# viridityzhu/HiFiHR

Measured on AMD Instinct MI355X. Metric: train images/sec, FreiHAND 224x224 (ResNet-18 + MANO LBS + render + losses + Adam), higher is better.
Workload: dtype f32; 1 GPU; BASELINE configs[1]: FreiHAND batch=32/GPU, ResNet-18 encoder + MANO LBS + silhouette/texture render losses, 224x224, aa=3 (672^2 samples); per_gpu_batch=32, global_batch=32, parallelism=dp1

## Files before the change

hifihr_amd/_lib.py:

```python
from __future__ import annotations

import ctypes
import os
from ctypes import POINTER, c_char_p, c_float, c_int, c_int32, c_long, c_size_t, c_void_p

import torch

_HERE = os.path.dirname(os.path.abspath(__file__))
LIB_PATH = os.path.join(_HERE, "libhifihr.so")

_c_float_p = POINTER(c_float)


class _LinearDesc(ctypes.Structure):
    _fields_ = [("x", c_void_p), ("w", c_void_p), ("b", c_void_p), ("y", c_void_p), ("B", c_int), ("I", c_int), ("O", c_int), ("act", c_int),
                ("dy", c_void_p), ("dz_scratch", c_void_p), ("dW_acc", c_void_p), ("db_acc", c_void_p), ("dx", c_void_p)]

_c_int_p = POINTER(c_int32)


class HifihrError(RuntimeError):
    pass


# ... 104 lines not shown
        c.hifihr_image_scale_to_nhwc4.argtypes = [_c_float_p, _c_float_p, c_int, c_int, c_int, _c_float_p, _c_float_p, c_void_p]
        c.hifihr_maxpool2d_fwd_notap.argtypes = [_c_float_p] + [c_int] * 7 + [_c_float_p, c_void_p]
        c.hifihr_lpips_tap_max_channels.argtypes = []
        c.hifihr_lpips_tap_max_channels.restype = c_int
        c.hifihr_lpips_tap_partial_floats.argtypes = [c_int]
        c.hifihr_lpips_tap_partial_floats.restype = c_size_t
        c.hifihr_lpips_tap.argtypes = [_c_float_p] * 3 + [c_int] * 4 + [_c_float_p, _c_float_p, c_void_p]
        c.hifihr_lpips_tap_bwd.argtypes = [_c_float_p] * 4 + [c_int] * 4 + [_c_float_p, c_void_p]
        c.hifihr_lpips_tap_bwd_relu.argtypes = [_c_float_p] * 4 + [c_int] * 4 + [_c_float_p, c_void_p]
        c.hifihr_lpips_maxpool_fwd.argtypes = [_c_float_p] + [c_int] * 4 + [_c_float_p, c_void_p]
        c.hifihr_lpips_maxpool_bwd.argtypes = [_c_float_p, _c_float_p] + [c_int] * 4 + [_c_float_p, c_void_p]
        c.hifihr_image_scale_to_nhwc4_bwd.argtypes = [_c_float_p, _c_float_p, c_int, c_int, c_int, _c_float_p, c_void_p]
        c.hifihr_geom_loss_fwd.argtypes = [_c_float_p] * 6 + [_c_int_p] + [c_int] * 7 + [_c_float_p] * 3 + [c_void_p]
        c.hifihr_geom_loss_bwd.argtypes = [_c_float_p] * 6 + [_c_int_p] * 3 + [c_int] * 7 + [_c_float_p] * 6 + [c_void_p]
        c.hifihr_photo_loss_partial_floats.argtypes = []
        c.hifihr_photo_loss_partial_floats.restype = c_int
        c.hifihr_photo_loss_fwd.argtypes = [_c_float_p, _c_float_p, c_void_p, c_int, c_int, c_int, c_float, c_float, c_float] + \
            [_c_float_p] * 4 + [c_void_p]
        c.hifihr_photo_loss_bwd.argtypes = [_c_float_p] * 6 + [c_int, c_int, c_int, c_float, c_float, _c_float_p, c_void_p]
        c.hifihr_sil_post.argtypes = [_c_float_p, _c_float_p, c_int, c_int, c_int, _c_float_p, _c_float_p, c_void_p]
        c.hifihr_linear_fwd.argtypes = [_c_float_p] * 3 + [c_int] * 4 + [_c_float_p] * 2 + [c_float, c_float] + [_c_float_p] * 6 + [c_void_p]
        c.hifihr_linear_bwd.argtypes = [_c_float_p] * 4 + [c_int] * 4 + [_c_float_p] * 10 + [c_void_p]
        c.hifihr_linear_fwd_group.argtypes = [POINTER(_LinearDesc), c_int, c_void_p]
        c.hifihr_linear_bwd_group.argtypes = [POINTER(_LinearDesc), c_int, c_void_p]
        c.hifihr_conv2d_bwd_data_pre.argtypes = [_c_float_p] * 3 + [c_int] * 9 + [c_void_p, c_size_t, c_void_p]
        c.hifihr_conv2d_bwd_data_pre_res.argtypes = [_c_float_p] * 4 + [c_int] * 9 + [c_void_p, c_size_t, c_void_p]
        c.hifihr_conv2d_bwd_data_pre_plus1x1.argtypes = [_c_float_p] * 5 + [c_int] * 9 + [c_void_p]
        c.hifihr_conv2d_bwd_data_pre_plus1x1_supported.argtypes = [c_int] * 9
        c.hifihr_conv2d_bwd_weight_plus1x1.argtypes = [_c_float_p] * 5 + [c_int] * 9 + [c_void_p]
        c.hifihr_conv2d_bwd_weight_plus1x1_supported.argtypes = [c_int] * 9
        c.hifihr_weight_prep.argtypes = [c_void_p, c_int, c_int, c_void_p]
        c.hifihr_freihand_augment.argtypes = [c_void_p, c_void_p, _c_int_p, _c_int_p, c_int, c_int, c_int, _c_float_p, _c_float_p, c_void_p]
        c.hifihr_ho3d_workspace_bytes.argtypes = [c_int, c_int]
        c.hifihr_ho3d_workspace_bytes.restype = c_size_t
        c.hifihr_ho3d_batch.argtypes = ([c_void_p, c_void_p] + [_c_float_p] * 3 + [c_int, c_int, _c_int_p, c_int, c_int, c_void_p, c_size_t] +
                                        [_c_float_p] * 5 + [c_void_p])
        c.hifihr_freihand_batch.argtypes = ([c_void_p, c_void_p] + [_c_float_p] * 4 + [c_int, c_int, _c_int_p, c_int, c_int, c_int, _c_float_p,
                                            _c_float_p, c_void_p] + [_c_float_p] * 6 + [c_void_p, c_void_p])
        c.hifihr_freihand_batch_step.argtypes = ([c_void_p, c_void_p] + [_c_float_p] * 4 + [c_int, c_int, _c_int_p, c_int, c_int, c_int, _c_float_p,
                                                 _c_float_p, c_void_p] + [_c_float_p] * 6 + [c_void_p, c_int, c_float] + [_c_float_p] * 4 + [c_void_p])
        c.hifihr_light_split_fwd.argtypes = [_c_float_p, c_int, _c_float_p, _c_float_p, c_void_p]
        c.hifihr_light_split_bwd.argtypes = [_c_float_p, _c_float_p, _c_float_p, c_int, _c_float_p, c_void_p]
        c.hifihr_wino4_bwd_gemm_pair_supported.argtypes = [c_int] * 5
        c.hifihr_wino4_bwd_gemm_pair.argtypes = [_c_float_p] * 6 + [c_int] * 6 + [c_void_p]
        c.hifihr_loss_total_fwd.argtypes = [POINTER(_c_float_p), POINTER(c_int), c_int, _c_float_p, c_void_p]
        c.hifihr_loss_total_bwd.argtypes = [_c_float_p, POINTER(_c_float_p), POINTER(c_int), POINTER(c_int), c_int, c_void_p]
        c.hifihr_procrustes_error.argtypes = [_c_float_p, _c_float_p, c_int, c_int, _c_float_p, _c_float_p, c_void_p]
        c.hifihr_point_error_hist.argtypes = [_c_float_p, _c_float_p, c_void_p, c_int, c_int, POINTER(ctypes.c_double), c_int, _c_int_p, c_void_p,
                                              c_void_p]
        c.hifihr_fscore_counts.argtypes = [_c_float_p, _c_float_p, c_int, c_int, c_int, POINTER(ctypes.c_double), c_int, _c_int_p, c_void_p]
        c.hifihr_wino_wgrad_gemm.argtypes = [_c_float_p] * 3 + [c_int] * 5 + [c_void_p]
        c.hifihr_wino_dw_transform.argtypes = [_c_float_p, _c_float_p, c_int, c_int, c_int, c_void_p]
        c.hifihr_weight_transpose.argtypes = [_c_float_p, _c_float_p, c_int, c_int, c_int, c_void_p]
        c.hifihr_bgemm_nt.argtypes = [_c_float_p] * 3 + [c_int] * 4 + [c_void_p, c_size_t, c_void_p]
        c.hifihr_bgemm_nt_workspace_bytes.argtypes = [c_int] * 4
        c.hifihr_bgemm_nt_workspace_bytes.restype = c_size_t
        c.hifihr_renderer_set_light_mode.argtypes = [c_void_p, c_int]
        c.hifihr_texture_pca_fwd.argtypes = [_c_float_p] * 3 + [c_int, c_int, c_long, _c_float_p, c_void_p]
        c.hifihr_texture_pca_bwd.argtypes = [_c_float_p] * 2 + [c_int, c_int, c_long, _c_float_p, c_void_p]
        c.hifihr_comm_last_error.restype = c_char_p
        c.hifihr_comm_get_unique_id.argtypes = [c_void_p]
        c.hifihr_comm_init.argtypes = [POINTER(c_void_p), c_int, c_int, c_void_p]
        c.hifihr_comm_allreduce_f32.argtypes = [c_void_p, _c_float_p, c_size_t, c_void_p]
        c.hifihr_comm_broadcast_f32.argtypes = [c_void_p, _c_float_p, c_size_t, c_int, c_void_p]
        c.hifihr_comm_destroy.argtypes = [c_void_p]
        c.hifihr_wino_tile.argtypes = [c_int] * 5
        c.hifihr_wino_gemm_workspace_bytes.argtypes = [c_int] * 6
        c.hifihr_wino_gemm_workspace_bytes.restype = c_size_t
        c.hifihr_wino_weight_transform.argtypes = [_c_float_p, _c_float_p, c_int, c_int, c_int, c_int, c_void_p]
        c.hifihr_wino_input_transform.argtypes = [_c_float_p, _c_float_p] + [c_int] * 5 + [c_void_p]
        c.hifihr_wino_gemm.argtypes = [_c_float_p] * 3 + [c_int] * 6 + [c_void_p, c_size_t, c_void_p]
        c.hifihr_wino_output_transform.argtypes = [_c_float_p] * 3 + [c_int] * 5 + [c_void_p]
        c.hifihr_wino_output_transform_act.argtypes = [_c_float_p] * 3 + [c_int] * 6 + [c_void_p]
        c.hifihr_conv3x3_c64_wino_supported.argtypes = [c_int] * 5
        c.hifihr_conv3x3_c64_wino.argtypes = [c_void_p, c_void_p, c_void_p, c_int, c_void_p, c_void_p, c_int, c_int, c_int, c_void_p]
        c.hifihr_conv3x3_c64_wino_res.argtypes = [c_void_p, c_void_p, c_void_p, c_void_p, c_int, c_int, c_int, c_void_p]
        c.hifihr_conv3x3_c64_bwd_pair_supported.argtypes = [c_int] * 3
        c.hifihr_conv3x3_c64_bwd_pair.argtypes = [c_void_p] * 7 + [c_size_t] + [c_int] * 3 + [c_void_p]
        c.hifihr_conv3x3_c64_bwd_pair_slabs.argtypes = [c_void_p] * 6 + [c_size_t] + [c_int] * 3 + [c_void_p, c_void_p]
        c.hifihr_conv_halo_wgrad_reduce_multi.argtypes = [c_void_p, c_int, c_void_p]
        c.hifihr_wino_bn_input_supported.argtypes = [c_int, c_int]
        c.hifihr_wino_bn_input_transform.argtypes = [_c_float_p] * 7 + [c_int] * 5 + [c_float, c_float] + [_c_float_p] * 4 + [c_void_p]
        c.hifihr_wino_output_transform_bnred.argtypes = [_c_float_p] * 10 + [c_int] * 5 + [c_void_p]
        c.hifihr_wino_bn_bwd_dual_transform.argtypes = [_c_float_p] * 8 + [c_int] * 5 + [_c_float_p] * 2 + [c_void_p]
        c.hifihr_bn_bwd_apply.argtypes = [_c_float_p] * 5 + [c_long, c_int] + [_c_float_p] * 4 + [c_void_p]
        c.hifihr_joint_terms_fwd.argtypes = [_c_float_p] * 4 + [c_int] * 3 + [POINTER(c_float), _c_float_p, c_void_p]
        c.hifihr_joint_terms_bwd.argtypes = [_c_float_p] * 4 + [c_int] * 3 + [POINTER(c_float)] + [_c_float_p] * 3 + [c_void_p]
        c.hifihr_wino_dy_transform.argtypes = [_c_float_p] * 2 + [c_int] * 5 + [c_void_p]
        c.hifihr_wino_input_dy_transform.argtypes = [_c_float_p] * 3 + [c_int] * 5 + [c_void_p]
        c.hifihr_wino_wgrad_parts.argtypes = [c_int] * 6
        c.hifihr_wino_wgrad_gemm_parts.argtypes = [_c_float_p] * 3 + [c_int] * 7 + [c_void_p]
        c.hifihr_wino_dw_transform_parts.argtypes = [_c_float_p, c_int, _c_float_p, c_int, c_int, c_int, c_void_p]
        c.hifihr_bgemm_describe.argtypes = [c_int] * 5 + [ctypes.c_char_p, c_int]
        c.hifihr_conv2d_describe.argtypes = [c_int] * 10 + [ctypes.c_char_p, c_int]
        c.hifihr_bgemm_tn_parts.argtypes = [c_int] * 4
        c.hifihr_bgemm_tn.argtypes = [_c_float_p] * 3 + [c_int] * 5 + [c_void_p]
        c.hifihr_wino4_dw_transform_multi.argtypes = [c_void_p, c_int, c_void_p]
        c.hifihr_se_pool.argtypes = [_c_float_p, c_int, c_int, c_int, _c_float_p, c_void_p]
        c.hifihr_se_scale.argtypes = [_c_float_p, _c_float_p, _c_float_p, c_float, c_int, c_int, c_int, _c_float_p, c_void_p]
        c.hifihr_se_bwd_gate.argtypes = [_c_float_p, _c_float_p, c_int, c_int, c_int, _c_float_p, c_void_p]
        c.hifihr_se_mlp_supported.argtypes = [c_int, c_int]
        c.hifihr_wino_tiles.argtypes = [c_int] * 4
        c.hifihr_wino_tiles.restype = c_long
        c.hifihr_wino_tiles_computed.argtypes = [c_int] * 4
        c.hifihr_wino_tiles_computed.restype = c_long
        c.hifihr_zero_page_ready.argtypes = [c_void_p]
        c.hifihr_drop_connect_add.argtypes = [_c_float_p, _c_float_p, _c_float_p, c_float, c_int, c_size_t, _c_float_p, c_void_p]
        c.hifihr_se_mlp_fwd.argtypes = [_c_float_p] * 5 + [c_int] * 3 + [_c_float_p] * 4 + [c_void_p]
        c.hifihr_se_mlp_bwd.argtypes = [_c_float_p] * 7 + [c_int] * 3 + [_c_float_p] * 7 + [c_void_p]
        c.hifihr_mmpool_fwd.argtypes = [_c_float_p, _c_float_p, c_int, c_int, c_int, _c_float_p, _c_int_p, _c_float_p, _c_float_p, c_void_p]
        c.hifihr_mmpool_bwd.argtypes = [_c_float_p, _c_float_p, _c_int_p, _c_float_p, _c_float_p, c_int, c_int, c_int, _c_float_p,
                                        _c_float_p, c_void_p]
        c.hifihr_maxpool2d_fwd.argtypes = [_c_float_p] + [c_int] * 7 + [_c_float_p, c_void_p, c_void_p]
        c.hifihr_maxpool2d_bwd.argtypes = [_c_float_p, c_void_p] + [c_int] * 7 + [_c_float_p, c_void_p]
        c.hifihr_maxpool2d_fwd_flat.argtypes = [_c_float_p] + [c_int] * 7 + [_c_float_p, c_void_p, c_void_p]
        c.hifihr_maxpool2d_bwd_flat.argtypes = [_c_float_p, c_void_p] + [c_int] * 7 + [_c_float_p, c_void_p]
        c.hifihr_maxpool2d_bwd_relu.argtypes = [_c_float_p, c_void_p, _c_float_p] + [c_int] * 7 + [_c_float_p, c_void_p]
        c.hifihr_wino_output_transform_mask.argtypes = [_c_float_p] * 3 + [c_int] * 5 + [c_void_p]
        c.hifihr_adam_step.argtypes = [_c_float_p, _c_float_p, _c_float_p, _c_float_p, c_size_t, c_float, c_float, c_float,
                                       c_float, c_float, c_float, c_int, c_void_p]
        c.hifihr_adam_state_bytes.restype = c_size_t
        c.hifihr_adam_state_bytes.argtypes = []
        c.hifihr_adam_step_counted.argtypes = [_c_float_p, _c_float_p, _c_float_p, _c_float_p, c_size_t, c_float, c_float, c_float, c_void_p, c_void_p]
        c.hifihr_grad_guard_bytes.restype = c_size_t
        c.hifihr_grad_guard_bytes.argtypes = []
        c.hifihr_grad_norm_workspace_bytes.restype = c_size_t
        c.hifihr_grad_norm_workspace_bytes.argtypes = [c_size_t]
        c.hifihr_grad_norm.argtypes = [_c_float_p, c_size_t, c_float, c_float, c_void_p, c_void_p, c_void_p]
        c.hifihr_adam_step_guarded.argtypes = [_c_float_p, _c_float_p, _c_float_p, _c_float_p, c_size_t, c_float, c_float, c_float, c_float,
                                               c_float, c_float, c_int, c_void_p, c_void_p, c_void_p]
        c.hifihr_adam_step_dyn.argtypes = [_c_float_p, _c_float_p, _c_float_p, _c_float_p, c_size_t, c_float, c_float, c_float,
                                           c_float, c_float, _c_float_p, c_void_p]
        c.hifihr_renderer_destroy.argtypes = [c_void_p]
        c.hifihr_render_workspace_bytes.argtypes = [c_void_p, c_int]
        c.hifihr_render_workspace_bytes.restype = c_size_t
        c.hifihr_render_fwd.argtypes = [c_void_p, _c_float_p, _c_float_p, c_int, _c_float_p, _c_float_p, _c_float_p, c_int,
                                        _c_float_p, _c_int_p, c_void_p, c_void_p]
        c.hifihr_render_bwd.argtypes = [c_void_p, _c_float_p, _c_float_p, _c_float_p, _c_float_p, _c_int_p, _c_float_p, c_int,
                                        _c_float_p, _c_float_p, _c_float_p, _c_float_p, c_void_p, c_void_p]
        c.hifihr_soft_sil_workspace_bytes.argtypes = [c_void_p, c_int]
        c.hifihr_soft_sil_workspace_bytes.restype = c_size_t
        c.hifihr_soft_sil_fwd.argtypes = [c_void_p, _c_float_p, _c_float_p, c_int, c_float, c_float, _c_float_p, _c_float_p, c_void_p, c_void_p]
        c.hifihr_soft_sil_bwd.argtypes = [c_void_p, _c_float_p, _c_float_p, _c_float_p, _c_float_p, c_int, c_float, c_float, _c_float_p, c_void_p,
                                          c_void_p]
        c.hifihr_soft_sil_loss_fwd.argtypes = [_c_float_p, c_void_p, c_int, c_int, c_int, c_float, c_float, c_void_p, _c_float_p, c_void_p]
        c.hifihr_soft_sil_loss_bwd.argtypes = [_c_float_p, c_void_p, c_int, c_void_p, _c_float_p, c_int, c_int, c_float, c_float, _c_float_p,
                                               c_void_p]
        c.hifihr_mesh_topology_create.argtypes = [_c_int_p, c_int, c_int]
        c.hifihr_mesh_topology_create.restype = c_void_p
        c.hifihr_mesh_topology_destroy.argtypes = [c_void_p]
        c.hifihr_mesh_topology_counts.argtypes = [c_void_p, _c_int_p, _c_int_p, _c_int_p]
        c.hifihr_mesh_reg_partial_floats.argtypes = [c_void_p, c_int]
        c.hifihr_mesh_reg_partial_floats.restype = c_size_t
        c.hifihr_mesh_reg_fwd.argtypes = [c_void_p, _c_float_p, c_int, c_float, c_float, _c_float_p, _c_float_p, _c_float_p, c_void_p]
        c.hifihr_mesh_reg_bwd.argtypes = [c_void_p, _c_float_p, _c_float_p, _c_float_p, c_int, c_float, c_float, _c_float_p, c_void_p]
        c.hifihr_chamfer_geometry.argtypes = [_c_int_p, _c_int_p]
        c.hifihr_chamfer_geometry.restype = None
        c.hifihr_chamfer_workspace_bytes.argtypes = [c_int, c_int, c_int]
        c.hifihr_chamfer_workspace_bytes.restype = c_size_t
        c.hifihr_chamfer_fwd.argtypes = [_c_float_p, _c_float_p, c_int, c_int, c_int, c_float, c_float, _c_int_p, _c_int_p, c_void_p, c_void_p,
                                         c_void_p, _c_float_p, c_void_p, c_void_p]
        c.hifihr_chamfer_bwd.argtypes = [_c_float_p, _c_float_p, _c_int_p, _c_int_p, _c_float_p, c_int, c_int, c_int, c_float, c_float,
                                         _c_float_p, _c_float_p, c_void_p]
        c.hifihr_renderer_set_uv.argtypes = [c_void_p, _c_int_p, _c_float_p, c_int]
        c.hifihr_render_uv_scratch_bytes.argtypes = [c_void_p, c_int]
        c.hifihr_render_uv_scratch_bytes.restype = c_size_t
# ... 244 lines not shown

    def wino_tile(self, N, H, W, C, K):
        return int(self.c.hifihr_wino_tile(N, H, W, C, K))

    def wino_gemm_workspace_bytes(self, N, H, W, C, K, m=2):
        return int(self.c.hifihr_wino_gemm_workspace_bytes(N, H, W, C, K, m))

    def wino4_bwd_gemm_pair_supported(self, N, H, W, C, K):
        key = (N, H, W, C, K)
        hit = self._pair_ok.get(key)
        if hit is None:
            hit = self._pair_ok[key] = bool(self.c.hifihr_wino4_bwd_gemm_pair_supported(int(N), int(H), int(W), int(C), int(K)))
        return hit

    def wino4_bwd_gemm_pair(self, V2, U2, M2, Vx, Yt, dU_parts, N, H, W, C, K, parts):
        self.check(self.c.hifihr_wino4_bwd_gemm_pair(_fp(V2), _fp(U2), _fp(M2), _fp(Vx), _fp(Yt), _fp(dU_parts), N, H, W, C, K, int(parts),
                                                     _stream_of(V2)), "hifihr_wino4_bwd_gemm_pair")

    def wino_weight_transform(self, w, U, K, C, flip, m=2):
        self.check(self.c.hifihr_wino_weight_transform(_fp(w), _fp(U), K, C, int(flip), m, _stream_of(w)), "hifihr_wino_weight_transform")

    def wino_input_transform(self, x, V, N, H, W, C, m=2):
        self.check(self.c.hifihr_wino_input_transform(_fp(x), _fp(V), N, H, W, C, m, _stream_of(x)), "hifihr_wino_input_transform")

    def zero_page_ready(self, device=None):
        import torch
        idx = torch.cuda.current_device() if device is None else torch.device(device).index
        idx = torch.cuda.current_device() if idx is None else idx
        if idx in self._zero_page:
            return True
        with torch.cuda.device(idx):
            ok = bool(self.c.hifihr_zero_page_ready(c_void_p(torch.cuda.current_stream(idx).cuda_stream)))
        if ok:
            self._zero_page.add(idx)
        return ok

    def conv3x3_c64_wino_supported(self, N, H, W, C, K):
        return bool(self.c.hifihr_conv3x3_c64_wino_supported(int(N), int(H), int(W), int(C), int(K)))

    def conv3x3_c64_wino(self, x, U, bias, relu, y, stats, N, H, W):
        self.check(self.c.hifihr_conv3x3_c64_wino(_fp(x), _fp(U), _fp(bias), int(bool(relu)), _fp(y), _fp(stats), N, H, W, _stream_of(x)),
                   "hifihr_conv3x3_c64_wino")

    def conv3x3_c64_wino_res(self, x, U, res, y, N, H, W):
        self.check(self.c.hifihr_conv3x3_c64_wino_res(_fp(x), _fp(U), _fp(res), _fp(y), N, H, W, _stream_of(x)), "hifihr_conv3x3_c64_wino_res")

    def conv3x3_c64_bwd_pair_supported(self, N, H, W):
        return bool(self.c.hifihr_conv3x3_c64_bwd_pair_supported(int(N), int(H), int(W)))

    def conv3x3_c64_bwd_pair(self, dy, U_bwd, res, dx, x, dw, N, H, W, ws=None):
        self.check(self.c.hifihr_conv3x3_c64_bwd_pair(_fp(dy), _fp(U_bwd), _fp(res), _fp(dx), _fp(x), _fp(dw), _fp(ws),
                                                      0 if ws is None else ws.numel() * ws.element_size(), N, H, W, _stream_of(dy)),
                   "hifihr_conv3x3_c64_bwd_pair")

    def conv3x3_c64_bwd_pair_slabs(self, dy, U_bwd, res, dx, x, slabs, N, H, W):
        import ctypes
        n = ctypes.c_int(0)
        self.check(self.c.hifihr_conv3x3_c64_bwd_pair_slabs(_fp(dy), _fp(U_bwd), _fp(res), _fp(dx), _fp(x), _fp(slabs), slabs.numel() * slabs.element_size(),
                                                            N, H, W, ctypes.cast(ctypes.pointer(n), c_void_p), _stream_of(dy)), "hifihr_conv3x3_c64_bwd_pair_slabs")
        return n.value

    def conv_halo_wgrad_reduce_multi(self, jobs):
        import ctypes
        import struct
        raw = b"".join(struct.pack("<QQii", sl.data_ptr(), dw.data_ptr(), int(n), 0) for sl, n, dw in jobs)
        buf = ctypes.create_string_buffer(raw, len(raw))
        self.check(self.c.hifihr_conv_halo_wgrad_reduce_multi(ctypes.cast(buf, c_void_p), len(jobs), _stream_of(jobs[0][0])),
                   "hifihr_conv_halo_wgrad_reduce_multi")

    def wino_bn_input_supported(self, C, m):
        return bool(self.c.hifihr_wino_bn_input_supported(int(C), int(m)))

    def wino_bn_input_transform(self, x, stats, gamma, beta, residual, out, V, N, H, W, C, m, eps, momentum, save_mean, save_invstd,
                                running_mean, running_var):
        self.check(self.c.hifihr_wino_bn_input_transform(_fp(x), _fp(stats), _fp(gamma), _fp(beta), _fp(residual), _fp(out), _fp(V), N, H, W, C, m,
                                                         eps, momentum, _fp(save_mean), _fp(save_invstd), _fp(running_mean), _fp(running_var),
                                                         _stream_of(x)), "hifihr_wino_bn_input_transform")

    def wino_output_transform_bnred(self, Mm, x, out, gadd, save_mean, save_invstd, gamma, beta, red, g, N, H, W, C, m):
        self.check(self.c.hifihr_wino_output_transform_bnred(_fp(Mm), _fp(x), _fp(out), _fp(gadd), _fp(save_mean), _fp(save_invstd), _fp(gamma),
                                                             _fp(beta), _fp(red), _fp(g), N, H, W, C, m, _stream_of(Mm)),
                   "hifihr_wino_output_transform_bnred")

    def wino_bn_bwd_dual_transform(self, g, y, save_mean, save_invstd, gamma, red, V, Yt, N, H, W, K, m, dgamma_acc, dbeta_acc):
        self.check(self.c.hifihr_wino_bn_bwd_dual_transform(_fp(g), _fp(y), _fp(save_mean), _fp(save_invstd), _fp(gamma), _fp(red), _fp(V), _fp(Yt),
                                                            N, H, W, K, m, _fp(dgamma_acc), _fp(dbeta_acc), _stream_of(g)),
                   "hifihr_wino_bn_bwd_dual_transform")

    def bn_bwd_apply(self, g, x, save_mean, save_invstd, gamma, M, C, red, dx, dgamma_acc, dbeta_acc):
        self.check(self.c.hifihr_bn_bwd_apply(_fp(g), _fp(x), _fp(save_mean), _fp(save_invstd), _fp(gamma), M, C, _fp(red), _fp(dx),
                                              _fp(dgamma_acc), _fp(dbeta_acc), _stream_of(g)), "hifihr_bn_bwd_apply")

    def wino_gemm(self, V, U, M, N, H, W, C, K, ws=None, m=2):
        self.check(self.c.hifihr_wino_gemm(_fp(V), _fp(U), _fp(M), N, H, W, C, K, m, *self._ws(ws), _stream_of(V)), "hifihr_wino_gemm")

    def wino_input_dy_transform(self, dy, V, Yt, N, H, W, K, m=2):
        self.check(self.c.hifihr_wino_input_dy_transform(_fp(dy), _fp(V), _fp(Yt), N, H, W, K, m, _stream_of(dy)), "hifihr_wino_input_dy_transform")

    def conv2d_bwd_data_pre(self, dy, wt, dx, N, H, W, C, K, R, S, stride, pad, ws=None):
        wsp, wsb = self._ws(ws)
        self.check(self.c.hifihr_conv2d_bwd_data_pre(_fp(dy), _fp(wt), _fp(dx), N, H, W, C, K, R, S, stride, pad, wsp, wsb, _stream_of(dy)),
                   "hifihr_conv2d_bwd_data_pre")

    def conv2d_bwd_data_pre_res(self, dy, wt, res, dx, N, H, W, C, K, R, S, stride, pad, ws=None):
        wsp, wsb = self._ws(ws)
        self.check(self.c.hifihr_conv2d_bwd_data_pre_res(_fp(dy), _fp(wt), _fp(res), _fp(dx), N, H, W, C, K, R, S, stride, pad, wsp, wsb,
                                                         _stream_of(dy)), "hifihr_conv2d_bwd_data_pre_res")

    def conv2d_bwd_data_pre_plus1x1_supported(self, N, H, W, C, K, R, S, stride, pad):
        return bool(self.c.hifihr_conv2d_bwd_data_pre_plus1x1_supported(int(N), int(H), int(W), int(C), int(K), int(R), int(S), int(stride), int(pad)))

    def conv2d_bwd_data_pre_plus1x1(self, dy, wt, dy2, wt2, dx, N, H, W, C, K, R, S, stride, pad):
        self.check(self.c.hifihr_conv2d_bwd_data_pre_plus1x1(_fp(dy), _fp(wt), _fp(dy2), _fp(wt2), _fp(dx), N, H, W, C, K, R, S, stride, pad,
                                                             _stream_of(dy)), "hifihr_conv2d_bwd_data_pre_plus1x1")

    def conv2d_bwd_weight_plus1x1_supported(self, N, H, W, C, K, R, S, stride, pad):
        return bool(self.c.hifihr_conv2d_bwd_weight_plus1x1_supported(int(N), int(H), int(W), int(C), int(K), int(R), int(S), int(stride), int(pad)))

    def conv2d_bwd_weight_plus1x1(self, x, dy, dw, dy2, dw2, N, H, W, C, K, R, S, stride, pad):
        self.check(self.c.hifihr_conv2d_bwd_weight_plus1x1(_fp(x), _fp(dy), _fp(dw), _fp(dy2), _fp(dw2), N, H, W, C, K, R, S, stride, pad,
                                                           _stream_of(x)), "hifihr_conv2d_bwd_weight_plus1x1")

    @staticmethod
    def prep_jobs(jobs, device):
        import struct
        raw = b"".join(struct.pack("<QQiiii", s.data_ptr(), d.data_ptr(), K, C, RS, kind) for s, d, K, C, RS, kind in jobs)
        return torch.frombuffer(bytearray(raw), dtype=torch.uint8).to(device)

    def weight_prep(self, table, njobs, blocks_per_job=64):
        self.check(self.c.hifihr_weight_prep(c_void_p(table.data_ptr()), njobs, blocks_per_job, _stream_of(table)), "hifihr_weight_prep")

    def freihand_batch(self, img_rgbx, mask, Ks, joints, verts, scales, packed, B, out, root_id=None, image_size=None):
        n, H, W = img_rgbx.shape
        J, V = joints.shape[1], verts.shape[1]
        vp = lambda t: c_void_p(t.data_ptr()) if t is not None else c_void_p(0)
        g = out.get
        for k in ("segms_gt", "idxs"):
            assert g(k) is None or g(k).dtype == torch.int64
        for t in out.values():
            assert t.is_contiguous()
        if root_id is None:
            self.check(self.c.hifihr_freihand_batch(vp(img_rgbx), vp(mask), _fp(Ks), _fp(joints), _fp(verts), _fp(scales), J, V, _ip(packed), B, H, W,
                                                    _fp(g("imgs")), _fp(g("masks")), vp(g("segms_gt")), _fp(g("Ks")), _fp(g("Ps")), _fp(g("joints")),
                                                    _fp(g("verts")), _fp(g("j2d_gt")), _fp(g("scales")), vp(g("idxs")), _stream_of(img_rgbx)),
                       "hifihr_freihand_batch")
            return
        self.check(self.c.hifihr_freihand_batch_step(vp(img_rgbx), vp(mask), _fp(Ks), _fp(joints), _fp(verts), _fp(scales), J, V, _ip(packed), B, H, W,
                                                     _fp(g("imgs")), _fp(g("masks")), vp(g("segms_gt")), _fp(g("Ks")), _fp(g("Ps")), _fp(g("joints")),
                                                     _fp(g("verts")), _fp(g("j2d_gt")), _fp(g("scales")), vp(g("idxs")), int(root_id), float(image_size or H),
                                                     _fp(g("root_xyz")), _fp(g("joints_rel")), _fp(g("verts_rel")), _fp(g("cam_ndc")), _stream_of(img_rgbx)),
                   "hifihr_freihand_batch_step")

    def ho3d_workspace_bytes(self, B, out_size):
        return int(self.c.hifihr_ho3d_workspace_bytes(B, out_size))

    def ho3d_batch(self, img_rgbx, hand_mask, Ks, uv21, xyz21, packed, B, out_size, ws, out):
        n, FH, FW = img_rgbx.shape
        vp = lambda t: c_void_p(t.data_ptr()) if t is not None else c_void_p(0)
        g = out.get
        for t in out.values():
            assert t.is_contiguous() and t.dtype == torch.float32
        self.check(self.c.hifihr_ho3d_batch(vp(img_rgbx), vp(hand_mask), _fp(Ks), _fp(uv21), _fp(xyz21), FH, FW, _ip(packed), B, out_size,
                                            vp(ws), c_size_t(ws.numel() * ws.element_size()), _fp(g("img_crop")), _fp(g("hand_mask_crop")),
                                            _fp(g("K_crop")), _fp(g("uv21_crop")), _fp(g("xyz21")), _stream_of(img_rgbx)), "hifihr_ho3d_batch")

    def freihand_augment(self, img_rgbx, mask, idx, coef_fix, out_img, out_mask):
# ... 500 lines not shown
```

hifihr_amd/csrc/bn_fold.h:

```cpp
#pragma once
#include <hip/hip_runtime.h>

#include "hifihr_internal.h"

namespace hifihr {

__device__ __forceinline__ bool last_workgroup(unsigned* __restrict__ cnt) {
  __shared__ int s_last;
  __syncthreads();
  if (threadIdx.x == 0) {
    const unsigned slot = blockIdx.x & 31u, nslots = gridDim.x < 32u ? gridDim.x : 32u;
    const unsigned in_slot = (gridDim.x + 31u - slot) / 32u;
    int last = 0;
    if (atomicAdd(cnt + slot, 1u) == in_slot - 1u) last = (atomicAdd(cnt + 32, 1u) == nslots - 1u) ? 1 : 0;
    s_last = last;
  }
  __syncthreads();
  return s_last != 0;
}

__device__ __forceinline__ void clear_slots(float* __restrict__ buf, int C, unsigned* __restrict__ cnt) {
  float4* p = reinterpret_cast<float4*>(buf);
  const int n4 = stat_slots_used(C) * 2 * C / 4;
  for (int i = threadIdx.x; i < n4; i += 256) p[i] = make_float4(0.f, 0.f, 0.f, 0.f);
  if (threadIdx.x < 33) cnt[threadIdx.x] = 0u;
}

template <int NS>
__device__ __forceinline__ void slot_sum2_n(const float* __restrict__ buf, int C, int c, float& s0, float& s1) {
  float a[NS], b[NS];
#pragma unroll
  for (int sl = 0; sl < NS; ++sl) { a[sl] = buf[(size_t)sl * 2 * C + c]; b[sl] = buf[(size_t)sl * 2 * C + C + c]; }
  s0 = 0.f; s1 = 0.f;
#pragma unroll
  for (int sl = 0; sl < NS; ++sl) { s0 += a[sl]; s1 += b[sl]; }
}
#if defined(HIFIHR_HOSTSIM)
#define HIFIHR_NO_HOIST() ((void)0)
#else
#define HIFIHR_NO_HOIST() asm volatile("" ::: "memory")
#endif
__device__ __forceinline__ void slot_sum2(const float* __restrict__ buf, int C, int c, float& s0, float& s1) {
  const int ns = stat_slots_used(C);
  if (ns == kStatSlots) { HIFIHR_NO_HOIST(); slot_sum2_n<kStatSlots>(buf, C, c, s0, s1); }
  else if (ns == 16) { HIFIHR_NO_HOIST(); slot_sum2_n<16>(buf, C, c, s0, s1); }
  else { HIFIHR_NO_HOIST(); slot_sum2_n<8>(buf, C, c, s0, s1); }
}

template <int NS>
__device__ __forceinline__ void slot_sums_fwd_n(const double* __restrict__ buf, int C, int c, double& s0, double& s1) {
  double a[NS], b[NS];
#pragma unroll
  for (int sl = 0; sl < NS; ++sl) { a[sl] = buf[(size_t)sl * 2 * C + c]; b[sl] = buf[(size_t)sl * 2 * C + C + c]; }
  s0 = 0.0; s1 = 0.0;
#pragma unroll
  for (int sl = 0; sl < NS; ++sl) { s0 += a[sl]; s1 += b[sl]; }
}
__device__ __forceinline__ void slot_mean_var(const float* __restrict__ stats, int C, int c, long M, float& mu, float& var) {
  const double* buf = reinterpret_cast<const double*>(stats);
  double s0, s1;
  const int ns = stat_slots_used(C);
  if (ns == kStatSlots) { HIFIHR_NO_HOIST(); slot_sums_fwd_n<kStatSlots>(buf, C, c, s0, s1); }
  else if (ns == 16) { HIFIHR_NO_HOIST(); slot_sums_fwd_n<16>(buf, C, c, s0, s1); }
  else { HIFIHR_NO_HOIST(); slot_sums_fwd_n<8>(buf, C, c, s0, s1); }
  const double m = s0 / (double)M;
  const double v = s1 / (double)M - m * m;
  mu = (float)m;
  var = v > 0.0 ? (float)v : 0.f;
}
__device__ __forceinline__ void clear_slots_fwd(float* __restrict__ stats, int C, unsigned* __restrict__ cnt) {
  float4* p = reinterpret_cast<float4*>(stats);
  const int n4 = stat_slots_used(C) * 2 * C / 2;
  for (int i = threadIdx.x; i < n4; i += 256) p[i] = make_float4(0.f, 0.f, 0.f, 0.f);
  if (threadIdx.x < 33) cnt[threadIdx.x] = 0u;
}

}
```

hifihr_amd/csrc/hifihr_api.hip:

```cpp
#include <hip/hip_runtime.h>

#include <algorithm>
#include <array>
#include <cmath>
#include <cstdarg>
#include <cstdio>
#include <cstring>
#include <new>
#include <vector>

#include "../../include/hifihr.h"
#include "hifihr_internal.h"
#include "mano_math.h"

namespace {

thread_local char g_err[512] = "";

int fail(int code, const char* fmt, ...) {
  va_list ap;
  va_start(ap, fmt);
  vsnprintf(g_err, sizeof(g_err), fmt, ap);
  va_end(ap);
  return code;
// ... 1522 lines not shown
  const WinoPlan p = wino_plan(N, H, W, m);
  if (parts != wino_tn_parts(p, C, K))
    return fail(HIFIHR_EINVAL, "hifihr_wino_wgrad_gemm_parts: parts must be hifihr_wino_wgrad_parts(N, H, W, C, K, m) > 0");
  HIP_TRY(hifihr::launch_bgemm_tn(Y, V, dU_parts, K, C, (int)p.T, p.P, parts, (hipStream_t)stream, (int)p.Tr));
  return HIFIHR_OK;
}

int hifihr_wino_dw_transform_parts(const float* dU_parts, int parts, float* dw_acc, int K, int C, int m, void* stream) {
  if (!dU_parts || !dw_acc || parts <= 0 || K <= 0 || C < 4 || C % 4 != 0 || !wino_m_ok(m))
    return fail(HIFIHR_EINVAL, "hifihr_wino_dw_transform_parts: bad argument");
  if (m == 4) HIP_TRY(hifihr::launch_wino4_dw_transform_parts(dU_parts, parts, dw_acc, K, C, (hipStream_t)stream));
  else HIP_TRY(hifihr::launch_wino_dw_transform_parts(dU_parts, parts, dw_acc, K, C, (hipStream_t)stream));
  return HIFIHR_OK;
}

int hifihr_wino4_dw_transform_multi(const hifihr_wino_dw_job* jobs, int njobs, void* stream) {
  static_assert(sizeof(hifihr_wino_dw_job) == sizeof(hifihr::WinoDwJob), "job layouts");
  if (!jobs || njobs <= 0) return fail(HIFIHR_EINVAL, "hifihr_wino4_dw_transform_multi: bad argument");
  for (int i = 0; i < njobs; ++i)
    if (!jobs[i].du_parts_d || !jobs[i].dw_acc_d || jobs[i].parts < 1 || jobs[i].K <= 0 || jobs[i].C < 4 || jobs[i].C % 4 != 0)
      return fail(HIFIHR_EINVAL, "hifihr_wino4_dw_transform_multi: bad job (pointers, parts >= 1, K > 0, C % 4 == 0)");
  HIP_TRY(hifihr::launch_wino4_dw_transform_multi(reinterpret_cast<const hifihr::WinoDwJob*>(jobs), njobs, (hipStream_t)stream));
  return HIFIHR_OK;
}

int hifihr_wino4_bwd_gemm_pair_supported(int N, int H, int W, int C, int K) {
  const WinoPlan p = wino_plan(N, H, W, 4);
  if (!wino_nt_ok(p, C, K) || !wino_tn_ok(p, C, K)) return 0;
  return hifihr::bgemm_nt_tn_pair_supported((int)p.Tr, (int)p.T, C, K, 36, K, C, (int)p.T, 36, wino_tn_parts(p, C, K)) ? 1 : 0;
}

int hifihr_wino4_bwd_gemm_pair(const float* V2, const float* U2, float* M2, const float* Vx, const float* Yt, float* dU_parts, int N, int H,
                               int W, int C, int K, int parts, void* stream) {
  const WinoPlan p = wino_plan(N, H, W, 4);
  if (!V2 || !U2 || !M2 || !Vx || !Yt || !dU_parts || parts <= 0 || !wino_nt_ok(p, C, K) || parts != wino_tn_parts(p, C, K))
    return fail(HIFIHR_EINVAL, "hifihr_wino4_bwd_gemm_pair: bad argument (C, K % 64 == 0; parts = hifihr_wino_wgrad_parts(N, H, W, C, K, 4))");
  if (!hifihr::bgemm_nt_fits32(p.T, C, K)) return fail(HIFIHR_EINVAL, "hifihr_wino4_bwd_gemm_pair: T * K and C * K must stay below 2^31 elements");
  const int T = (int)p.T, Tr = (int)p.Tr;
  const hipError_t e = hifihr::launch_bgemm_nt_tn_pair(V2, U2, M2, Tr, T, C, K, 36, Yt, Vx, dU_parts, K, C, T, 36, parts, (hipStream_t)stream, Tr);
  if (e == hipSuccess) return HIFIHR_OK;
  if (e != hipErrorNotSupported) HIP_TRY(e);
  HIP_TRY(hifihr::launch_bgemm_nt(V2, U2, M2, Tr, C, K, 36, nullptr, 0, (hipStream_t)stream, nullptr, T));
  HIP_TRY(hifihr::launch_bgemm_tn(Yt, Vx, dU_parts, K, C, T, 36, parts, (hipStream_t)stream, Tr));
  return HIFIHR_OK;
}

int hifihr_wino_wgrad_gemm(const float* V, const float* Y, float* dU_zeroed, int N, int H, int W, int C, int K, void* stream) {
  const WinoPlan p = wino_plan(N, H, W, 2);
  if (!V || !Y || !dU_zeroed || !p.ok || C < 4 || C % 4 != 0 || K < 4 || K % 4 != 0)
    return fail(HIFIHR_EINVAL, "hifihr_wino_wgrad_gemm: bad argument (C % 4 == 0, K % 4 == 0)");
  HIP_TRY(hifihr::launch_conv_wgrad(wino_gemm_geom(p.T, C, K), V, Y, dU_zeroed, nullptr, 0, (hipStream_t)stream));
  return HIFIHR_OK;
}

int hifihr_wino_dw_transform(float* dU, float* dw_acc, int K, int C, int clear_du, void* stream) {
  if (!dU || !dw_acc || K <= 0 || C < 4 || C % 4 != 0) return fail(HIFIHR_EINVAL, "hifihr_wino_dw_transform: bad argument");
  HIP_TRY(hifihr::launch_wino_dw_transform(dU, dw_acc, K, C, clear_du ? 1 : 0, (hipStream_t)stream));
  return HIFIHR_OK;
}

int hifihr_wino_bn_input_supported(int C, int m) { return (m == 4 && hifihr::wino4_bn_supported(C)) ? 1 : 0; }

int hifihr_wino_bn_input_transform(const float* x, float* stats, const float* gamma, const float* beta, const float* residual, float* out,
                                   float* V, int N, int H, int W, int C, int m, float eps, float momentum, float* save_mean,
                                   float* save_invstd, float* running_mean, float* running_var, void* stream) {
  if (!x || !stats || !gamma || !beta || !V || !save_mean || !save_invstd || N <= 0 || H <= 0 || W <= 0 || ((residual == nullptr) != (out == nullptr)))
    return fail(HIFIHR_EINVAL, "hifihr_wino_bn_input_transform: bad argument");
  if (!hifihr_wino_bn_input_supported(C, m)) return fail(HIFIHR_EINVAL, "hifihr_wino_bn_input_transform: needs m = 4 and C % 4 == 0, C <= 512");
  HIP_TRY(hifihr::launch_wino4_bn_input_transform(x, stats, gamma, beta, residual, out, V, N, H, W, C, eps, momentum, save_mean, save_invstd,
                                                  running_mean, running_var, (hipStream_t)stream));
  return HIFIHR_OK;
}

int hifihr_wino_output_transform_bnred(const float* Mm, const float* x, const float* out, const float* gadd, const float* save_mean,
                                       const float* save_invstd, const float* gamma, const float* beta, float* red, float* g, int N, int H, int W,
                                       int C, int m, void* stream) {
  if (!Mm || !x || !save_mean || !save_invstd || !gamma || !beta || !red || !g || N <= 0 || H <= 0 || W <= 0)
    return fail(HIFIHR_EINVAL, "hifihr_wino_output_transform_bnred: bad argument");
  if (!hifihr_wino_bn_input_supported(C, m)) return fail(HIFIHR_EINVAL, "hifihr_wino_output_transform_bnred: needs m = 4 and C % 4 == 0, C <= 512");
  HIP_TRY(hifihr::launch_wino4_output_transform_bnred(Mm, x, out, gadd, save_mean, save_invstd, gamma, beta, red, g, N, H, W, C, (hipStream_t)stream));
  return HIFIHR_OK;
}

int hifihr_wino_bn_bwd_dual_transform(const float* g, const float* y, const float* save_mean, const float* save_invstd, const float* gamma,
                                      float* red, float* V, float* Yt, int N, int H, int W, int K, int m, float* dgamma_acc, float* dbeta_acc,
                                      void* stream) {
  if (!g || !y || !save_mean || !save_invstd || !gamma || !red || !V || !Yt || N <= 0 || H <= 0 || W <= 0)
    return fail(HIFIHR_EINVAL, "hifihr_wino_bn_bwd_dual_transform: bad argument");
  if (!hifihr_wino_bn_input_supported(K, m)) return fail(HIFIHR_EINVAL, "hifihr_wino_bn_bwd_dual_transform: needs m = 4 and K % 4 == 0, K <= 512");
  HIP_TRY(hifihr::launch_wino4_bn_bwd_dual_transform(g, y, save_mean, save_invstd, gamma, red, V, Yt, N, H, W, K, dgamma_acc, dbeta_acc,
                                                     (hipStream_t)stream));
  return HIFIHR_OK;
}

int hifihr_bn_bwd_apply(const float* g, const float* x, const float* save_mean, const float* save_invstd, const float* gamma, long M, int C,
                        float* red, float* dx, float* dgamma_acc, float* dbeta_acc, void* stream) {
  if (!g || !x || !save_mean || !save_invstd || !gamma || !red || !dx || M <= 0 || C < 4 || C % 4 != 0 || C > 512)
    return fail(HIFIHR_EINVAL, "hifihr_bn_bwd_apply: bad argument (C % 4 == 0, C <= 512)");
  HIP_TRY(hifihr::launch_bn_bwd_apply(g, x, save_mean, save_invstd, gamma, M, C, red, dx, dgamma_acc, dbeta_acc, (hipStream_t)stream));
  return HIFIHR_OK;
}

int hifihr_conv3x3_c64_wino_supported(int N, int H, int W, int C, int K) { return hifihr::conv_wino2_supported(N, H, W, C, K) ? 1 : 0; }

int hifihr_zero_page_ready(void* stream) { return hifihr::conv_halo_zero_page((hipStream_t)stream) != nullptr ? 1 : 0; }

int hifihr_conv3x3_c64_wino(const float* x, const float* u, const float* bias, int relu, float* y, float* stats, int N, int H, int W, void* stream) {
  if (!x || !u || !y) return fail(HIFIHR_EINVAL, "hifihr_conv3x3_c64_wino: null pointer");
  if (!hifihr::conv_wino2_supported(N, H, W, 64, 64))
    return fail(HIFIHR_EINVAL, "hifihr_conv3x3_c64_wino: needs even H and even W >= 14 (or HIFIHR_CONV_WINO2=0 is set)");
  HIP_TRY(hifihr::launch_conv_wino2(x, u, bias, relu, y, stats, N, H, W, (hipStream_t)stream));
  return HIFIHR_OK;
}

int hifihr_conv3x3_c64_wino_res(const float* x, const float* u, const float* res, float* y, int N, int H, int W, void* stream) {
  if (!x || !u || !y || !res) return fail(HIFIHR_EINVAL, "hifihr_conv3x3_c64_wino_res: null pointer");
  if (!hifihr::conv_wino2_supported(N, H, W, 64, 64))
    return fail(HIFIHR_EINVAL, "hifihr_conv3x3_c64_wino_res: needs even H and even W >= 14 (or HIFIHR_CONV_WINO2=0 is set)");
  HIP_TRY(hifihr::launch_conv_wino2(x, u, nullptr, 0, y, nullptr, N, H, W, (hipStream_t)stream, res));
  return HIFIHR_OK;
}

int hifihr_conv3x3_c64_bwd_pair_supported(int N, int H, int W) { return hifihr::conv_c64_bwd_pair_supported(N, H, W) ? 1 : 0; }

int hifihr_conv3x3_c64_bwd_pair(const float* dy, const float* u_bwd, const float* res, float* dx, const float* x, float* dw, void* ws,
                                size_t ws_bytes, int N, int H, int W, void* stream) {
  if (!dy || !u_bwd || !dx || !x || !dw) return fail(HIFIHR_EINVAL, "hifihr_conv3x3_c64_bwd_pair: null pointer");
  if (!hifihr::conv_c64_bwd_pair_supported(N, H, W))
    return fail(HIFIHR_EINVAL, "hifihr_conv3x3_c64_bwd_pair: unsupported shape (ask hifihr_conv3x3_c64_bwd_pair_supported)");
  HIP_TRY(hifihr::launch_conv_c64_bwd_pair(dy, u_bwd, res, dx, x, dw,
                                           (ws && ws_bytes >= hifihr::conv_halo_wgrad_slab_bytes()) ? static_cast<float*>(ws) : nullptr, N, H, W,
                                           (hipStream_t)stream));
  return HIFIHR_OK;
}

int hifihr_conv3x3_c64_bwd_pair_slabs(const float* dy, const float* u_bwd, const float* res, float* dx, const float* x, void* slabs, size_t slab_bytes,
                                      int N, int H, int W, int* nslab, void* stream) {
  if (!dy || !u_bwd || !dx || !x || !slabs || !nslab) return fail(HIFIHR_EINVAL, "hifihr_conv3x3_c64_bwd_pair_slabs: null pointer");
  if (!hifihr::conv_c64_bwd_pair_supported(N, H, W) || slab_bytes < hifihr::conv_halo_wgrad_slab_bytes())
    return fail(HIFIHR_EINVAL, "hifihr_conv3x3_c64_bwd_pair_slabs: unsupported shape, or fewer than hifihr_conv2d_wgrad_workspace_bytes slab bytes");
  HIP_TRY(hifihr::launch_conv_c64_bwd_pair(dy, u_bwd, res, dx, x, nullptr, static_cast<float*>(slabs), N, H, W, (hipStream_t)stream, nslab));
  return HIFIHR_OK;
}

int hifihr_conv_halo_wgrad_reduce_multi(const hifihr_halo_reduce_job* jobs, int njobs, void* stream) {
  static_assert(sizeof(hifihr_halo_reduce_job) == sizeof(hifihr::HaloReduceJob), "job layouts");
  if (!jobs || njobs <= 0) return fail(HIFIHR_EINVAL, "hifihr_conv_halo_wgrad_reduce_multi: bad argument");
  for (int i = 0; i < njobs; ++i)
    if (!jobs[i].slabs_d || !jobs[i].dw_acc_d || jobs[i].nslab <= 0) return fail(HIFIHR_EINVAL, "hifihr_conv_halo_wgrad_reduce_multi: bad job");
  HIP_TRY(hifihr::launch_conv_halo_wgrad_reduce_multi(reinterpret_cast<const hifihr::HaloReduceJob*>(jobs), njobs, (hipStream_t)stream));
  return HIFIHR_OK;
}

int hifihr_freihand_augment(const uint32_t* img_rgbx, const uint8_t* mask, const int* idx, const int* coef_fix, int B, int H, int W,
                            float* out_img, float* out_mask, void* stream) {
  if (!idx || !coef_fix || (!out_img && !out_mask) || (out_img && !img_rgbx) || (out_mask && !mask) || B <= 0 || H <= 0 || W <= 0 ||
      (long)H * W >= (1L << 24))
    return fail(HIFIHR_EINVAL, "hifihr_freihand_augment: bad argument (H * W < 2^24)");
  HIP_TRY(hifihr::launch_freihand_augment(img_rgbx, mask, idx, coef_fix, B, H, W, out_img, out_mask, (hipStream_t)stream));
  return HIFIHR_OK;
}

int hifihr_freihand_batch(const uint32_t* img_rgbx, const uint8_t* mask, const float* Ks, const float* joints, const float* verts,
                          const float* scales, int J, int V, const int* packed, int B, int H, int W, float* out_img, float* out_mask,
                          long long* out_segm, float* out_Ks, float* out_Ps, float* out_joints, float* out_verts, float* out_j2d,
                          float* out_scales, long long* out_idxs, void* stream) {
// ... 66 lines not shown
```

hifihr_amd/csrc/hifihr_internal.h:

```cpp
#pragma once
#include <hip/hip_runtime.h>

#include <cstdint>
#include <cstdlib>
#include <stdint.h>

#include "render_math.h"

namespace hifihr {

inline int device_cus() {
  static int cus = 0;
  if (cus == 0) {
    int dev = 0;
    hipDeviceProp_t prop;
    if (hipGetDevice(&dev) == hipSuccess && hipGetDeviceProperties(&prop, dev) == hipSuccess && prop.multiProcessorCount > 0) cus = prop.multiProcessorCount;
  }
  return cus > 0 ? cus : 256;
}

static inline int env_int(const char* name, int unset) {
  const char* e = getenv(name);
  return e ? atoi(e) : unset;
}
// ... 339 lines not shown
  float *oroot, *ojoints_rel, *overts_rel, *ocam;
};
hipError_t launch_freihand_batch(const uint32_t* img, const uint8_t* mask, const float* Ks, const float* joints, const float* verts,
                                 const float* scales, int J, int V, const int* packed, int B, int H, int W, float* out_img, float* out_mask,
                                 long long* out_segm, float* oKs, float* oPs, float* ojoints, float* overts, float* oj2d, float* oscales,
                                 long long* oidx, const BatchStepOut& step, hipStream_t st);
size_t ho3d_workspace_bytes(int B, int out_size);
hipError_t launch_ho3d_batch(const uint32_t* img, const uint8_t* mask, const float* Ks, const float* uv21, const float* xyz21, int FH, int FW,
                             const int* packed, int B, int out_size, void* ws, float* out_img, float* out_mask, float* out_K,
                             float* out_uv, float* out_xyz, hipStream_t st);
hipError_t launch_procrustes(const float* pred, const float* gt, int B, int N, float* aligned, float* err_sum, hipStream_t st);
constexpr int kHistMaxT = 128, kFscoreMaxT = 8;
struct HistThresholds { double v[kHistMaxT]; };
struct FscoreThresholds { double v[kFscoreMaxT]; };
bool thresholds_ok(const double* thr_h, int T, bool positive);
hipError_t launch_point_error_hist(const float* pred, const float* gt, const unsigned char* vis, int n, int K, const double* thr_h, int T,
                                   int* hist, double* sum, hipStream_t st);
hipError_t launch_fscore_counts(const float* pred, const float* gt, int B, int Np, int Ng, const double* thr_h, int T, int* counts,
                                hipStream_t st);
hipError_t launch_wino_output_transform(const float* Mm, float* y, float* stats, const float* bias, int relu, int N, int H, int W, int K,
                                        hipStream_t st);
hipError_t launch_wino_dy_transform(const float* dy, float* Y, int N, int H, int W, int K, hipStream_t st);
hipError_t launch_wino_dw_transform(float* dU, float* dw, int K, int C, int clear, hipStream_t st);

struct BgemmArgs {
  const float* A; const float* B; float* C;
  int M, N, K;
  int lda, ldb, ldc;
  long sa, sb, sc;
  int batch, tiles_m, tiles_n;
  int splits, cps;
  long sc_split;
  const float* zeros = nullptr;
  int cIH = 0, cIW = 0, cC = 0, cOH = 0, cOW = 0, cR = 0, cS = 0, cStride = 1, cPad = 0;
  int co_r = 0, co_rounds = 0;
  int k_valid = 0;
  float* stats = nullptr;
};
void bgemm_describe(int tn, int M, int N, int K, char* out, int cap);
void bgemm_describe_batch(int tn, int M, int N, int K, int batch, char* out, int cap);
bool bgemm_nt_supported(int M, int N, int K);
bool bgemm_nt_fits32(long M_alloc, int N, int K);
bool bgemm_tn_supported(int M, int N, int T);
size_t bgemm_nt_workspace_bytes(int M, int N, int K, int batch);
bool bgemm_nt_stats_supported(int N);
bool conv_rows_supported(const ConvGeom& g, const float* bias);
hipError_t launch_conv_rows(const ConvGeom& g, const float* src, const float* wgt, float* dst, float* stats, const float* zeros, hipStream_t st);
bool conv_rows_pair_supported(const ConvGeom& g1, const ConvGeom& g2);
hipError_t launch_conv_rows_pair(const ConvGeom& g1, const float* src, const float* w1, float* y1, float* stats1, const ConvGeom& g2, const float* w2,
                                 float* y2, float* stats2, const float* zeros, hipStream_t st);
bool bgemm_nt_ragged_supported(int M, int N, int K);
enum class NtKernel { rows, rows_ragged, sk, ws, tile };
struct NtPlan {
  bool ok;
  NtKernel kernel;
  int M, M_alloc, N, K, batch;
  int bm, bn, loaders;
  int G;
  long per;
  size_t ws_bytes;
};
NtPlan plan_nt(int M, int M_alloc, int N, int K, int batch, bool stats);
void describe_nt(const NtPlan& p, char* out, int cap);
hipError_t launch_bgemm_nt_plan(const NtPlan& p, const float* A, const float* B, float* C, void* ws, size_t ws_bytes, hipStream_t st, float* stats_or_null);
hipError_t launch_bgemm_nt(const float* A, const float* B, float* C, int M, int N, int K, int batch, void* ws, size_t ws_bytes, hipStream_t st,
                           float* stats_or_null = nullptr, int M_alloc = 0);
int bgemm_tn_parts(int M, int N, int T, int batch);
hipError_t launch_bgemm_tn(const float* A, const float* B, float* Cparts, int M, int N, int T, int batch, int parts, hipStream_t st, int T_valid = 0);
bool bgemm_nt_tn_pair_supported(int M, int M_alloc, int N, int K, int batch, int M2, int N2, int T2, int batch2, int parts2);
hipError_t launch_bgemm_nt_tn_pair(const float* A, const float* B, float* C, int M, int M_alloc, int N, int K, int batch, const float* A2,
                                   const float* B2, float* C2parts, int M2, int N2, int T2, int batch2, int parts2, hipStream_t st, int T2_valid = 0);
hipError_t launch_wino_dw_transform_parts(const float* dU_parts, int parts, float* dw, int K, int C, hipStream_t st);
long wino4_tiles(int N, int H, int W);
long wino4_tiles_real(int N, int H, int W);
hipError_t launch_wino4_weight_transform(const float* w, float* U, int K, int C, int flip, hipStream_t st);
hipError_t launch_wino4_input_transform(const float* x, float* V, float* Y , int N, int H, int W, int C, hipStream_t st);
bool wino4_bn_supported(int C);
hipError_t launch_wino4_bn_input_transform(const float* x, float* stats, const float* gamma, const float* beta, const float* res, float* out,
                                           float* V, int N, int H, int W, int C, float eps, float momentum, float* save_mean,
                                           float* save_invstd, float* running_mean, float* running_var, hipStream_t st);
hipError_t launch_wino4_output_transform_bnred(const float* Mm, const float* x, const float* outp, const float* gadd, const float* save_mean,
                                               const float* save_invstd, const float* gamma, const float* beta, float* red, float* g, int N,
                                               int H, int W, int C, hipStream_t st);
hipError_t launch_wino4_bn_bwd_dual_transform(const float* g, const float* y, const float* save_mean, const float* save_invstd, const float* gamma,
                                              float* red, float* V, float* Y, int N, int H, int W, int K, float* dgamma_acc, float* dbeta_acc,
                                              hipStream_t st);
hipError_t launch_bn_bwd_apply(const float* g, const float* x, const float* save_mean, const float* save_invstd, const float* gamma, long M,
                               int C, float* red, float* dx, float* dgamma_acc, float* dbeta_acc, hipStream_t st);
hipError_t launch_wino4_output_transform(const float* Mm, float* y, float* stats, const float* bias, int relu, const float* mask, int N, int H, int W, int K,
                                         hipStream_t st);
hipError_t launch_wino4_dy_transform(const float* dy, float* Y, int N, int H, int W, int K, hipStream_t st);
hipError_t launch_wino4_dw_transform_parts(const float* dU_parts, int parts, float* dw, int K, int C, hipStream_t st);
struct WinoDwJob { const float* dU; float* dw; int parts, K, C; };
hipError_t launch_wino4_dw_transform_multi(const WinoDwJob* jobs, int njobs, hipStream_t st);

hipError_t launch_texpca_fwd(const float* coef, const float* basis, const float* mean, int B, int K, long n, float* out, hipStream_t st);
hipError_t launch_texpca_bwd(const float* g, const float* basis, int B, int K, long n, float* dcoef_zeroed, hipStream_t st);
size_t adam_state_bytes();
hipError_t launch_adam_counted(float* p, const float* g, float* m, float* v, size_t n, float grad_scale, float eps, float weight_decay,
                               void* state, hipStream_t st);
hipError_t launch_adam(float* p, const float* g, float* m, float* v, size_t n, float grad_scale, float lr, float beta1,
                       float beta2, float eps, float weight_decay, int step, const float* dyn, hipStream_t st);
size_t grad_guard_bytes();
size_t grad_norm_workspace_bytes(size_t n);
hipError_t launch_grad_norm(const float* g, size_t n, float grad_scale, float max_norm, void* guard, void* ws, hipStream_t st);
hipError_t launch_adam_guarded(float* p, const float* g, float* m, float* v, size_t n, float grad_scale, float lr, float beta1, float beta2,
                               float eps, float weight_decay, int step, void* state, const void* guard, hipStream_t st);

hipError_t launch_joint_terms_fwd(const float* j2d, const float* j2d_gt, const float* j3d, const float* j3d_gt, int B, int J, int mse,
                                  const float* lam3, float* out3, hipStream_t st);
hipError_t launch_joint_terms_bwd(const float* j2d, const float* j2d_gt, const float* j3d, const float* j3d_gt, int B, int J, int mse,
                                  const float* lam3, const float* gout3, float* g_j2d, float* g_j3d, hipStream_t st);

}
```

hifihr_amd/csrc/wino4_bn.hip:

```cpp
#include <hip/hip_runtime.h>

#include <cstdlib>

#include "bn_fold.h"
#include "hifihr_internal.h"
#include "wino4_math.h"

namespace hifihr {

using namespace w4;

TileGeo wino4_geo(int N, int H, int W);

constexpr int kWbnMaxC = 512;

__device__ __forceinline__ V4 relu0(const V4& z) { return V4{fmaxf(z.x, 0.f), fmaxf(z.y, 0.f), fmaxf(z.z, 0.f), fmaxf(z.w, 0.f)}; }
__device__ __forceinline__ float relu0(float z) { return fmaxf(z, 0.f); }

template <typename T>
__device__ __forceinline__ T bn_res_relu(const T& v, const T& sc, const T& sh, const T& r, bool has_res) {
  T z = v * sc + sh;
  if (has_res) z = z + r;
  return relu0(z);
}

template <bool RES, typename T>
struct WbnPatch {
  T v[6][6];
  T r[RES ? 6 : 1][RES ? 6 : 1];
  unsigned long long ok;
  int cg;
  size_t t;
  size_t own[4][4];
};

template <bool RES, typename T>
__device__ __forceinline__ void wbn_load(WbnPatch<RES, T>& p, size_t i, const float* __restrict__ x, const float* __restrict__ res,
                                         const TileGeo& geo, int C) {
  constexpr int VW = VecWidth<T>::n;
  const int CV = C / VW;
  p.cg = (int)(i % CV);
  p.t = i / CV;
  const TileAt at = tile_at(geo, p.t);
    const AxisBase by_ = axis_base(geo, at.y0, geo.H), bx_ = axis_base(geo, at.x0, geo.W);
  AxisPx ry[6];
#pragma unroll
  for (int r = 0; r < 6; ++r) ry[r] = row_px(geo, at, by_, r - 1);
  p.ok = 0ull;
#pragma unroll
  for (int c = 0; c < 6; ++c) {
    const AxisPx cx = col_px(geo, bx_, c - 1);
#pragma unroll
    for (int r = 0; r < 6; ++r) {
      bool ok;
      const size_t px = tile_pixel(ry[r], cx, ok);
      const size_t o = px * C + p.cg * VW;
      p.v[r][c] = ldT<T>(x + o);
      if constexpr (RES) {
        p.r[r][c] = ldT<T>(res + o);
        if (r >= 1 && r <= 4 && c >= 1 && c <= 4) p.own[r - 1][c - 1] = px;
      }
      p.ok |= ok ? (1ull << (6 * r + c)) : 0ull;
    }
  }
}

template <bool RES, typename T>
__device__ __forceinline__ void wbn_emit(const WbnPatch<RES, T>& p, const float* s_sc, const float* s_sh, float* __restrict__ out,
                                         float* __restrict__ V, int C, size_t Tn) {
  constexpr int VW = VecWidth<T>::n;
  const T sc = ldT<T>(&s_sc[p.cg * VW]), sh = ldT<T>(&s_sh[p.cg * VW]);
  T tt[6][6];
#pragma unroll
  for (int c = 0; c < 6; ++c) {
    T col[6];
#pragma unroll
    for (int r = 0; r < 6; ++r) {
      const bool ok = (p.ok >> (6 * r + c)) & 1ull;
      const T a = bn_res_relu<T>(p.v[r][c], sc, sh, RES ? p.r[RES ? r : 0][RES ? c : 0] : zeroT<T>(), RES);
      col[r] = ok ? a : zeroT<T>();
      if (RES && r >= 1 && r <= 4 && c >= 1 && c <= 4 && ok)
        stT(out + p.own[RES ? r - 1 : 0][RES ? c - 1 : 0] * C + p.cg * VW, a);
    }
    T o[6];
    bt6(col, o);
#pragma unroll
    for (int r = 0; r < 6; ++r) tt[r][c] = o[r];
  }
#pragma unroll
  for (int r = 0; r < 6; ++r) {
    T o[6];
    bt6(tt[r], o);
#pragma unroll
    for (int c = 0; c < 6; ++c) stT(V + ((size_t)(r * 6 + c) * Tn + p.t) * C + p.cg * VW, o[c]);
  }
}

template <bool RES, typename T, bool MOS>
__global__ __launch_bounds__(256) void wino4_bn_input_transform_kernel(const float* __restrict__ x, float* __restrict__ stats,
                                                                         const float* __restrict__ gamma, const float* __restrict__ beta,
                                                                         const float* __restrict__ res, float* __restrict__ out,
                                                                         float* __restrict__ V, TileGeo geo, int C,
                                                                         float eps, float momentum, float* __restrict__ save_mean,
                                                                         float* __restrict__ save_invstd, float* __restrict__ running_mean,
                                                                         float* __restrict__ running_var) {
  if (!MOS) geo.G = 0;
  __shared__ float s_sc[kWbnMaxC], s_sh[kWbnMaxC];
  const long M = (long)geo.N * geo.H * geo.W;
  const size_t Tn = tile_count(geo), total = Tn * (C / VecWidth<T>::n);
  for (int c = threadIdx.x; c < C; c += 256) {
    float mu, var;
    slot_mean_var(stats, C, c, M, mu, var);
    const float is = 1.0f / sqrtf(var + eps);
    const float sc = is * gamma[c];
    s_sc[c] = sc;
    s_sh[c] = beta[c] - mu * sc;
    if (blockIdx.x == 0) {
      save_mean[c] = mu;
      save_invstd[c] = is;
      if (running_mean) {
        running_mean[c] = (1.f - momentum) * running_mean[c] + momentum * mu;
        const float unbiased = (M > 1) ? var * ((float)M / (float)(M - 1)) : var;
        running_var[c] = (1.f - momentum) * running_var[c] + momentum * unbiased;
      }
    }
  }
  __syncthreads();
  for (size_t i = (size_t)blockIdx.x * 256 + threadIdx.x; i < total; i += (size_t)gridDim.x * 256) {
    WbnPatch<RES, T> p;
    wbn_load<RES, T>(p, i, x, res, geo, C);
    wbn_emit<RES, T>(p, s_sc, s_sh, out, V, C, Tn);
  }
  unsigned* cnt = stat_fwd_counters(stats, C);
  if (last_workgroup(cnt)) clear_slots_fwd(stats, C, cnt);
}

template <bool RES, bool ADD, bool MOS>
__global__ __launch_bounds__(256) void wino4_output_transform_bnred_kernel(const float* __restrict__ Mm, const float* __restrict__ x,
                                                                          const float* __restrict__ outp, const float* __restrict__ gadd,
                                                                          const float* __restrict__ save_mean, const float* __restrict__ save_invstd,
                                                                          const float* __restrict__ gamma, const float* __restrict__ beta,
                                                                          float* __restrict__ red, float* __restrict__ g, TileGeo geo, int C) {
  if (!MOS) geo.G = 0;
  __shared__ float4 redl[2][16][16];
  const int cl = threadIdx.x & 15, tl = threadIdx.x >> 4;
  const int k = blockIdx.y * 64 + cl * 4;
  const bool kok = k < C;
  const size_t T = tile_count(geo);
  V4 sg = zero4(), sq = zero4();
  if (kok) {
    const V4 mu = ld4(save_mean + k), is = ld4(save_invstd + k), ga = ld4(gamma + k), be = ld4(beta + k);
    const V4 sc = V4{is.x * ga.x, is.y * ga.y, is.z * ga.z, is.w * ga.w};
    const V4 sh = V4{be.x - mu.x * sc.x, be.y - mu.y * sc.y, be.z - mu.z * sc.z, be.w - mu.w * sc.w};
    for (size_t t = (size_t)blockIdx.x * 16 + tl; t < T; t += (size_t)gridDim.x * 16) {
      const TileAt at = tile_at(geo, t);
    const AxisBase by_ = axis_base(geo, at.y0, geo.H), bx_ = axis_base(geo, at.x0, geo.W);
      AxisPx cx[4];
#pragma unroll
      for (int b = 0; b < 4; ++b) cx[b] = col_px(geo, bx_, b);
      V4 s[4][6];
#pragma unroll
      for (int c = 0; c < 6; ++c) {
        V4 col[6];
#pragma unroll
        for (int r = 0; r < 6; ++r) col[r] = ld4(Mm + ((size_t)(r * 6 + c) * T + t) * C + k);
        V4 o[4];
        at6(col, o);
#pragma unroll
        for (int a = 0; a < 4; ++a) s[a][c] = o[a];
      }
#pragma unroll
      for (int a = 0; a < 4; ++a) {
        const AxisPx ry = row_px(geo, at, by_, a);
        if (ry.ok) {
          V4 xv[4], ov[4], av[4];
          bool ok[4];
          size_t ob[4];
#pragma unroll
          for (int b = 0; b < 4; ++b) {
            ob[b] = tile_pixel(ry, cx[b], ok[b]) * C + k;
            const size_t o = ob[b];
            xv[b] = ld4(x + o);
            ov[b] = RES ? ld4(outp + o) : zero4();
            av[b] = ADD ? ld4(gadd + o) : zero4();
          }
          V4 o[4];
          at6(s[a], o);
#pragma unroll
          for (int b = 0; b < 4; ++b) {
            if (ok[b]) {
              V4 d = o[b];
              if (ADD) d = d + av[b];
              V4 z;
              if (RES) z = ov[b];
              else z = V4{xv[b].x * sc.x + sh.x, xv[b].y * sc.y + sh.y, xv[b].z * sc.z + sh.z, xv[b].w * sc.w + sh.w};
              const V4 gm = V4{z.x > 0.f ? d.x : 0.f, z.y > 0.f ? d.y : 0.f, z.z > 0.f ? d.z : 0.f, z.w > 0.f ? d.w : 0.f};
              st4(g + ob[b], gm);
              sg = sg + gm;
              sq.x += gm.x * ((xv[b].x - mu.x) * is.x); sq.y += gm.y * ((xv[b].y - mu.y) * is.y);
              sq.z += gm.z * ((xv[b].z - mu.z) * is.z); sq.w += gm.w * ((xv[b].w - mu.w) * is.w);
            }
          }
        }
      }
    }
  }
  redl[0][tl][cl] = make_float4(sg.x, sg.y, sg.z, sg.w); redl[1][tl][cl] = make_float4(sq.x, sq.y, sq.z, sq.w);
  __syncthreads();
  if (tl == 0 && kok) {
    float4 a1 = redl[0][0][cl], a2 = redl[1][0][cl];
    for (int r = 1; r < 16; ++r) {
      const float4 b1 = redl[0][r][cl], b2 = redl[1][r][cl];
      a1 = make_float4(a1.x + b1.x, a1.y + b1.y, a1.z + b1.z, a1.w + b1.w);
      a2 = make_float4(a2.x + b2.x, a2.y + b2.y, a2.z + b2.z, a2.w + b2.w);
    }
    float* sp = red + (size_t)(blockIdx.x & (stat_slots_used(C) - 1)) * 2 * C;
    atomicAdd(sp + k, a1.x); atomicAdd(sp + k + 1, a1.y); atomicAdd(sp + k + 2, a1.z); atomicAdd(sp + k + 3, a1.w);
    atomicAdd(sp + C + k, a2.x); atomicAdd(sp + C + k + 1, a2.y); atomicAdd(sp + C + k + 2, a2.z); atomicAdd(sp + C + k + 3, a2.w);
  }
}

template <typename T, bool MOS>
__global__ __launch_bounds__(256) void wino4_bn_bwd_dual_transform_kernel(const float* __restrict__ g, const float* __restrict__ y,
                                                                         const float* __restrict__ save_mean, const float* __restrict__ save_invstd,
                                                                         const float* __restrict__ gamma, float* __restrict__ red,
                                                                         float* __restrict__ V, float* __restrict__ Y, TileGeo geo, int K,
                                                                         float* __restrict__ dgamma_acc, float* __restrict__ dbeta_acc) {
  constexpr int VW = VecWidth<T>::n;
  if (!MOS) geo.G = 0;
  __shared__ float s_mg[kWbnMaxC], s_mgx[kWbnMaxC];
  const float invM = 1.0f / (float)((long)geo.N * geo.H * geo.W);
  for (int c = threadIdx.x; c < K; c += 256) {
    float sgv, sgx;
    slot_sum2(red, K, c, sgv, sgx);
    s_mg[c] = sgv * invM;
    s_mgx[c] = sgx * invM;
    if (blockIdx.x == 0) {
      if (dgamma_acc) dgamma_acc[c] += sgx;
      if (dbeta_acc) dbeta_acc[c] += sgv;
    }
  }
  __syncthreads();
  const int KV = K / VW;
  const size_t Tn = tile_count(geo), total = Tn * KV;
  for (size_t i = (size_t)blockIdx.x * 256 + threadIdx.x; i < total; i += (size_t)gridDim.x * 256) {
    const int cg = (int)(i % KV);
    const size_t t = i / KV;
    const TileAt at = tile_at(geo, t);
    const AxisBase by_ = axis_base(geo, at.y0, geo.H), bx_ = axis_base(geo, at.x0, geo.W);
    AxisPx ry[6];
#pragma unroll
    for (int r = 0; r < 6; ++r) ry[r] = row_px(geo, at, by_, r - 1);
    const T mu = ldT<T>(save_mean + cg * VW), is = ldT<T>(save_invstd + cg * VW), ga = ldT<T>(gamma + cg * VW);
    const T k1 = is * ga;
    const T mg = ldT<T>(&s_mg[cg * VW]), mgx = ldT<T>(&s_mgx[cg * VW]);
    T tt[6][6];
    T ty[6][4];
#pragma unroll
    for (int c = 0; c < 6; ++c) {
      const AxisPx cx = col_px(geo, bx_, c - 1);
      T col[6], yv[6];
      bool okr[6];
#pragma unroll
      for (int r = 0; r < 6; ++r) {
        const size_t o = tile_pixel(ry[r], cx, okr[r]) * K + cg * VW;
        col[r] = ldT<T>(g + o);
        yv[r] = ldT<T>(y + o);
      }
#pragma unroll
      for (int r = 0; r < 6; ++r) {
        const T d = k1 * (col[r] - mg - (yv[r] - mu) * is * mgx);
        col[r] = okr[r] ? d : zeroT<T>();
      }
      T o[6];
      bt6(col, o);
#pragma unroll
      for (int r = 0; r < 6; ++r) tt[r][c] = o[r];
      if (c >= 1 && c <= 4) {
        T o2[6];
        a4(col + 1, o2);
#pragma unroll
        for (int r = 0; r < 6; ++r) ty[r][c - 1] = o2[r];
      }
    }
#pragma unroll
    for (int r = 0; r < 6; ++r) {
      T o[6];
      bt6(tt[r], o);
#pragma unroll
      for (int c = 0; c < 6; ++c) stT(V + ((size_t)(r * 6 + c) * Tn + t) * K + cg * VW, o[c]);
    }
#pragma unroll
    for (int r = 0; r < 6; ++r) {
      T o[6];
      a4(ty[r], o);
#pragma unroll
      for (int c = 0; c < 6; ++c) stT(Y + ((size_t)(r * 6 + c) * Tn + t) * K + cg * VW, o[c]);
    }
  }
  unsigned* cnt = stat_bwd_counters(red, K);
  if (last_workgroup(cnt)) clear_slots(red, K, cnt);
}

static unsigned wbn_grid(size_t total) {
  size_t b = (total + 255) / 256;
  if (b > 4096) b = 4096;
  if (b < 1) b = 1;
  return (unsigned)b;
}

static bool wbn_scalar(size_t items_v4) { return items_v4 < (size_t)256 * 2048; }

bool wino4_bn_supported(int C) { return C >= 4 && C % 4 == 0 && C <= kWbnMaxC; }

hipError_t launch_wino4_bn_input_transform(const float* x, float* stats, const float* gamma, const float* beta, const float* res, float* out,
                                           float* V, int N, int H, int W, int C, float eps, float momentum, float* save_mean,
                                           float* save_invstd, float* running_mean, float* running_var, hipStream_t st) {
  if (!wino4_bn_supported(C) || ((res == nullptr) != (out == nullptr))) return hipErrorInvalidValue;
  const TileGeo geo = wino4_geo(N, H, W);
  const size_t total = tile_count(geo) * (C / 4);
#define HIFIHR_WBN_IN2(R_, M_)                                                                                                                 \
  hipLaunchKernelGGL((wino4_bn_input_transform_kernel<R_, V4, M_>), dim3(wbn_grid(total)), dim3(256), 0, st, x, stats, gamma, beta, res, out, V, \
                     geo, C, eps, momentum, save_mean, save_invstd, running_mean, running_var)
#define HIFIHR_WBN_IN(R_) { if (geo.G) HIFIHR_WBN_IN2(R_, true); else HIFIHR_WBN_IN2(R_, false); }
  if (res != nullptr) HIFIHR_WBN_IN(true) else HIFIHR_WBN_IN(false)
#undef HIFIHR_WBN_IN
#undef HIFIHR_WBN_IN2
  return hipGetLastError();
}

hipError_t launch_wino4_output_transform_bnred(const float* Mm, const float* x, const float* outp, const float* gadd, const float* save_mean,
                                               const float* save_invstd, const float* gamma, const float* beta, float* red, float* g, int N,
                                               int H, int W, int C, hipStream_t st) {
  if (!wino4_bn_supported(C)) return hipErrorInvalidValue;
  const TileGeo geo = wino4_geo(N, H, W);
  const size_t T = tile_count(geo);
  size_t bx = (T + 15) / 16;
  if (bx > 1024) bx = 1024;
  const dim3 grid((unsigned)bx, (C + 63) / 64);
#define HIFIHR_BNRED2(R_, A_, M_)                                                                                                          \
  hipLaunchKernelGGL((wino4_output_transform_bnred_kernel<R_, A_, M_>), grid, dim3(256), 0, st, Mm, x, outp, gadd, save_mean, save_invstd, gamma, \
                     beta, red, g, geo, C)
#define HIFIHR_BNRED(R_, A_) { if (geo.G) HIFIHR_BNRED2(R_, A_, true); else HIFIHR_BNRED2(R_, A_, false); }
  if (outp != nullptr) {
    if (gadd != nullptr) HIFIHR_BNRED(true, true) else HIFIHR_BNRED(true, false)
  } else {
    if (gadd != nullptr) HIFIHR_BNRED(false, true) else HIFIHR_BNRED(false, false)
  }
#undef HIFIHR_BNRED
#undef HIFIHR_BNRED2
  return hipGetLastError();
}

hipError_t launch_wino4_bn_bwd_dual_transform(const float* g, const float* y, const float* save_mean, const float* save_invstd, const float* gamma,
                                              float* red, float* V, float* Y, int N, int H, int W, int K, float* dgamma_acc, float* dbeta_acc,
                                              hipStream_t st) {
  if (!wino4_bn_supported(K)) return hipErrorInvalidValue;
  const TileGeo geo = wino4_geo(N, H, W);
  const size_t total = tile_count(geo) * (K / 4);
#define HIFIHR_WBN_DUAL(T_, M_, TOT_)                                                                                                       \
  hipLaunchKernelGGL((wino4_bn_bwd_dual_transform_kernel<T_, M_>), dim3(wbn_grid(TOT_)), dim3(256), 0, st, g, y, save_mean, save_invstd, gamma, \
                     red, V, Y, geo, K, dgamma_acc, dbeta_acc)
  if (wbn_scalar(total)) { if (geo.G) HIFIHR_WBN_DUAL(float, true, total * 4); else HIFIHR_WBN_DUAL(float, false, total * 4); }
  else { if (geo.G) HIFIHR_WBN_DUAL(V4, true, total); else HIFIHR_WBN_DUAL(V4, false, total); }
#undef HIFIHR_WBN_DUAL
  return hipGetLastError();
}

}
```

hifihr_amd/network.py:

```python
from __future__ import annotations

import torch
import torch.nn as nn
import torch.nn.functional as F
from torch.nn import init


def weights_init(m):
    name = m.__class__.__name__
    if name.find("Block") == -1 and name.find("Conv") != -1:
        init.kaiming_normal_(m.weight.data, a=0, mode="fan_in")
    elif name.find("Linear") != -1:
        init.kaiming_normal_(m.weight.data, a=0, mode="fan_in")
    elif name.find("BatchNorm") != -1:
        init.normal_(m.weight.data, 1.0, 0.02)
    if hasattr(m, "bias") and m.bias is not None:
        init.constant_(m.bias.data, 0.0)


class Conv2dMFMA(nn.Module):

    def __init__(self, cin, cout, k, stride=1, pad=0, bias=False, relu=True):
        super().__init__()
        self.stride, self.pad, self.relu = stride, pad, relu
        self.weight = nn.Parameter(torch.empty(cout, cin, k, k).contiguous(memory_format=torch.channels_last))
        init.kaiming_uniform_(self.weight, a=5 ** 0.5)
        self.bias = None
        if bias:
            bound = 1.0 / (cin * k * k) ** 0.5
            self.bias = nn.Parameter(torch.empty(cout).uniform_(-bound, bound))

    def forward(self, x, want_stats=False, grad_premasked=False, mask_input_grad=False, fork=False):
        from . import ops
        w = self.weight
        if self.bias is not None:
            return ops.conv2d_bias_act(x, w, self.bias, self.stride, self.pad, self.relu,
                                       grad_premasked=grad_premasked and not self.bias.requires_grad, mask_input_grad=mask_input_grad)
        return ops.conv2d(x, w, self.stride, self.pad, want_stats, fork)


def _conv(cin, cout, k, stride, pad):
    return Conv2dMFMA(cin, cout, k, stride, pad)


def _conv_bn(conv, x, bn):
    if bn.training:
        return conv(x, want_stats=True)
    return conv(x), None


def _conv_bn_fork(conv, x, bn):
    from . import ops
    if not (x.requires_grad and torch.is_grad_enabled() and ops.conv_fork_enabled()):
        out, st = _conv_bn(conv, x, bn)
        return out, st, x
    if bn.training:
        return conv(x, want_stats=True, fork=True)
    out, xa = conv(x, fork=True)
    return out, None, xa


class _PendingBN:

    def __init__(self, y, stats, bn, identity):
        self.y, self.stats, self.bn, self.identity = y, stats, bn, identity

    def materialize(self):
        from . import ops
        return ops.bn_act(self.y, self.stats, self.bn, self.identity, True)


def _resolve(x):
    return x.materialize() if isinstance(x, _PendingBN) else x


class BasicBlock(nn.Module):
    expansion = 1

    def __init__(self, inplanes, planes, stride=1, downsample=None):
        super().__init__()
        self.conv1 = _conv(inplanes, planes, 3, stride, 1)
        self.bn1 = nn.BatchNorm2d(planes)
        self.conv2 = _conv(planes, planes, 3, 1, 1)
        self.bn2 = nn.BatchNorm2d(planes)
        self.downsample = downsample
        self.lazy_out = False

    def forward(self, x):
        from . import ops
        idt_raw = st_ds = None
        fused = False
        if isinstance(x, _PendingBN):
            p = x
            if p.bn.training and ops.bn_wino_fusable(p.y, self.conv1.weight, p.bn, self.conv1.stride, self.conv1.pad):
                out, st, x = ops.bn_act_wino_conv(p.y, p.stats, p.bn, p.identity, self.conv1.weight, self.bn1.training)
                fused = True
            else:
                x = p.materialize()
        if not fused:
            ds = self.downsample
            if (ds is not None and self.bn1.training and ds[1].training and self.conv1.stride == 2 and torch.is_grad_enabled()
                    and ops.conv2d_pair_ok(x, self.conv1.weight, ds[0].weight, 2)):
                out, st, idt_raw, st_ds = ops.conv2d_pair(x, self.conv1.weight, ds[0].weight, 2)
            else:
                out, st, x = _conv_bn_fork(self.conv1, x, self.bn1)
        if st is not None and ops.bn_wino_fusable(out, self.conv2.weight, self.bn1, 1, 1):
            out, st, _ = ops.bn_act_wino_conv(out, st, self.bn1, None, self.conv2.weight, self.bn2.training)
        else:
            out = ops.bn_act(out, st, self.bn1, None, True)
            out, st = _conv_bn(self.conv2, out, self.bn2)
        idt = x
        if idt_raw is not None:
            idt = ops.bn_act(idt_raw, st_ds, self.downsample[1], None, False)
        elif self.downsample is not None:
            idt, st2 = _conv_bn(self.downsample[0], x, self.downsample[1])
            idt = ops.bn_act(idt, st2, self.downsample[1], None, False)
        if self.lazy_out and self.bn2.training:
            return _PendingBN(out, st, self.bn2, idt)
        return ops.bn_act(out, st, self.bn2, idt, True)


class Bottleneck(nn.Module):
    expansion = 4

    def __init__(self, inplanes, planes, stride=1, downsample=None):
        super().__init__()
        self.conv1 = _conv(inplanes, planes, 1, 1, 0)
        self.bn1 = nn.BatchNorm2d(planes)
        self.conv2 = _conv(planes, planes, 3, stride, 1)
        self.bn2 = nn.BatchNorm2d(planes)
        self.conv3 = _conv(planes, planes * 4, 1, 1, 0)
        self.bn3 = nn.BatchNorm2d(planes * 4)
        self.downsample = downsample

    def forward(self, x):
        from . import ops
        x = _resolve(x)
        out, st = _conv_bn(self.conv1, x, self.bn1)
        out = ops.bn_act(out, st, self.bn1, None, True)
        out, st = _conv_bn(self.conv2, out, self.bn2)
        out = ops.bn_act(out, st, self.bn2, None, True)
        out, st = _conv_bn(self.conv3, out, self.bn3)
        idt = x
        if self.downsample is not None:
            idt, st2 = _conv_bn(self.downsample[0], x, self.downsample[1])
            idt = ops.bn_act(idt, st2, self.downsample[1], None, False)
        return ops.bn_act(out, st, self.bn3, idt, True)


class ResNet18Trunk(nn.Module):
    block, layers = BasicBlock, (2, 2, 2, 2)

    def __init__(self, in_ch=3, layer4_stride=1, block=None, layers=None):
        super().__init__()
        if block is not None:
            self.block, self.layers = block, tuple(layers)
        self.conv1 = _conv(in_ch, 64, 7, 2, 3)
        self.bn1 = nn.BatchNorm2d(64)
        self.inplanes = 64
        self.layer1 = self._make(64, self.layers[0], 1)
        self.layer2 = self._make(128, self.layers[1], 2)
        self.layer3 = self._make(256, self.layers[2], 2)
        self.layer4 = self._make(512, self.layers[3], layer4_stride)
        for m in self.modules():
            if isinstance(m, Conv2dMFMA):
                init.kaiming_normal_(m.weight, mode="fan_out", nonlinearity="relu")

    def _make(self, planes, blocks, stride):
        blk, out = self.block, planes * self.block.expansion
        down = None
        if stride != 1 or self.inplanes != out:
            down = nn.Sequential(_conv(self.inplanes, out, 1, stride, 0), nn.BatchNorm2d(out))
        layers = [blk(self.inplanes, planes, stride, down)]
        self.inplanes = out
        layers += [blk(out, planes) for _ in range(1, blocks)]
        return nn.Sequential(*layers)


class Resnet_4C(nn.Module):
    def __init__(self, pretrain="res18", if_4c=False):
        super().__init__()
        arch = {"res18": (BasicBlock, (2, 2, 2, 2)), "res50": (Bottleneck, (3, 4, 6, 3)), "res101": (Bottleneck, (3, 4, 23, 3))}
        if pretrain not in arch:
            raise NotImplementedError(f"encoder '{pretrain}' is not built (res18 / res50 / res101; the HRNet variants need timm)")
        self.model = ResNet18Trunk(in_ch=4 if if_4c else 3, layer4_stride=1, block=arch[pretrain][0], layers=arch[pretrain][1])
        m = self.model
        blocks = [b for layer in (m.layer1, m.layer2, m.layer3, m.layer4) for b in layer]
        for b, nxt in zip(blocks, blocks[1:]):
            if isinstance(b, BasicBlock) and isinstance(nxt, BasicBlock) and b is not m.layer2[-1]:
                b.lazy_out = True

    def forward(self, x):
        from . import ops
        m = self.model
        h, st = _conv_bn(m.conv1, x, m.bn1)
        x = ops.bn_relu_maxpool(h, st, m.bn1)
        x = m.layer1(x)
        x_low = _resolve(m.layer2(x))
        cut = getattr(self, "segment_cut", None)
# ... 151 lines not shown
```

hifihr_amd/ops.py:

```python
from __future__ import annotations

import math
import os
import threading

import torch

from ._lib import get_lib, require_cuda


import os as _os

_DEBUG_SYNC = _os.environ.get("HIFIHR_DEBUG_SYNC", "0") == "1"


class _Profile:

    def __init__(self):
        self.on = False
        self.events = []
        self.last_render = None
        self.conv_log = []

    def enable(self):
# ... 1152 lines not shown
    def forward(ctx, x, w1, w2, stride):
        require_cuda(x, w1, w2)
        lib = get_lib()
        x = x.contiguous(memory_format=_CL)
        wk1, wk2 = w1.contiguous(memory_format=_CL), w2.contiguous(memory_format=_CL)
        N, C, H, W = x.shape
        K1, K2 = wk1.shape[0], wk2.shape[0]
        OH, OW = (H + 2 - 3) // stride + 1, (W + 2 - 3) // stride + 1
        y1 = torch.empty((N, K1, OH, OW), device=x.device, dtype=torch.float32, memory_format=_CL)
        y2 = torch.empty((N, K2, OH, OW), device=x.device, dtype=torch.float32, memory_format=_CL)
        st1 = _ZERO_POOL.acquire(lib.bn_stats_floats(K1), x.device)
        st2 = _ZERO_POOL.acquire(lib.bn_stats_floats(K2), x.device)
        if PROFILE.on:
            PROFILE.conv_log.append((("pair", N, H, W, C, K1, K2, stride), "fwd-pair"))
        PROFILE.bracket("conv_fwd", lambda: lib.conv2d_fwd_bnstats_pair(x, wk1, y1, st1, K1, 3, 1, wk2, y2, st2, K2, 1, 0, N, H, W, C, stride))
        ctx.geom1, ctx.geom2 = (N, H, W, C, K1, 3, 3, stride, 1), (N, H, W, C, K2, 1, 1, stride, 0)
        ctx.save_for_backward(x, wk1, wk2)
        ctx.w1, ctx.w2 = w1, w2
        ctx.wino_allowed = _wino_allowed()
        ctx.set_materialize_grads(False)
        ctx.mark_non_differentiable(st1, st2)
        return y1, st1, y2, st2

    @staticmethod
    def backward(ctx, gy1, _gs1, gy2, _gs2):
        x, wk1, wk2 = ctx.saved_tensors
        need_x, need_w1, need_w2 = ctx.needs_input_grad[0], ctx.needs_input_grad[1], ctx.needs_input_grad[2]

        def conv(gy, wk, geom, w, need_x, need_w, **kw):
            return _conv_backward(gy, x, wk, None, None, geom, w, need_x=need_x, need_w=need_w, wino_allowed=ctx.wino_allowed, **kw)
        N, H, W, C, K1, R, S, stride, pad = ctx.geom1
        plus = None
        if gy1 is not None and gy2 is not None and need_x and wk2.shape[0] == K1:
            lib = get_lib()
            if lib.conv2d_bwd_data_pre_plus1x1_supported(N, H, W, C, K1, R, S, stride, pad):
                wt1, wt2 = _WEIGHT_PREP.get(ctx.w1, wk1, 0), _WEIGHT_PREP.get(ctx.w2, wk2, 0)
                if wt1 is not None and wt2 is not None:
                    plus = (gy2.contiguous(memory_format=_CL), wt2)
        if plus is not None:
            w_both = (need_w1 and need_w2 and not _ASYNC_WGRAD.active
                      and lib.conv2d_bwd_weight_plus1x1_supported(N, H, W, C, K1, R, S, stride, pad))
            dw1 = dw2 = None
            if w_both:
                gy1c = gy1.contiguous(memory_format=_CL)
                t1, dw1 = _grad_target(ctx.w1, wk1, _CL)
                t2, dw2 = _grad_target(ctx.w2, wk2, _CL)
                if PROFILE.on:
                    PROFILE.conv_log.append((ctx.geom1, "wgrad+1x1"))
                PROFILE.bracket("conv_wgrad", lambda: lib.conv2d_bwd_weight_plus1x1(x, gy1c, t1, plus[0], t2, N, H, W, C, K1, R, S, stride, pad))
                if dw1 is None:
                    _grad_ready(ctx.w1)
                if dw2 is None:
                    _grad_ready(ctx.w2)
            else:
                dw2 = conv(gy2, wk2, ctx.geom2, ctx.w2, False, need_w2)[1]
            dx, dw1b, _ = conv(gy1, wk1, ctx.geom1, ctx.w1, need_x, need_w1 and not w_both, plus1x1=plus)
            return dx, (dw1 if w_both else dw1b), dw2, None
        dx2 = dw2 = dw1 = None
        if gy2 is not None:
            dx2, dw2, _ = conv(gy2, wk2, ctx.geom2, ctx.w2, need_x, need_w2)
        if gy1 is not None:
            dx, dw1, _ = conv(gy1, wk1, ctx.geom1, ctx.w1, need_x, need_w1, g_fork=dx2)
        else:
            dx = dx2
        return dx, dw1, dw2, None


def conv2d_pair_ok(x, w1, w2, stride):
    if not (x.is_cuda and torch.is_tensor(x) and w1.shape[2:] == (3, 3) and w2.shape[2:] == (1, 1) and w1.shape[1] == x.shape[1] == w2.shape[1]):
        return False
    lib = get_lib()
    N, C, H, W = x.shape
    return lib.zero_page_ready(x.device) and lib.conv2d_fwd_bnstats_pair_supported(N, H, W, C, stride, w1.shape[0], 3, 1, w2.shape[0], 1, 0)


def conv2d_pair(x, w1, w2, stride):
    return _Conv2dPair.apply(x, w1, w2, stride)


def conv_fork_enabled():
    return os.environ.get("HIFIHR_CONV_FORK", "1") != "0"


class _BNAct(torch.autograd.Function):
    @staticmethod
    def forward(ctx, x, stats, gamma, beta, residual, act, eps, momentum, running_mean, running_var):
        require_cuda(x, stats, gamma, beta)
        lib = get_lib()
        x = x.contiguous(memory_format=_CL)
        N, C, H, W = x.shape
        M = N * H * W
        res = residual.contiguous(memory_format=_CL) if residual is not None else None
        y = torch.empty_like(x, memory_format=_CL)
        save_mean = torch.empty(C, device=x.device)
        save_invstd = torch.empty(C, device=x.device)
        PROFILE.bracket("bn_fwd", lambda: lib.bn_act_fwd(x, stats, gamma, beta, res, act, M, C, eps, momentum, y, save_mean,
                                                         save_invstd, running_mean, running_var))
        _ZERO_POOL.release(stats)
        ctx.save_for_backward(x, y if (act == 1 and residual is not None) else x.new_empty(0), gamma, beta, save_mean, save_invstd)
        ctx.act, ctx.has_res, ctx.M, ctx.C = act, residual is not None, M, C
        ctx.gamma_param, ctx.beta_param = gamma, beta
        return y

    @staticmethod
    def backward(ctx, dy):
        x, y, gamma, beta, save_mean, save_invstd = ctx.saved_tensors
        dx, dg, db, dres = _bn_act_backward(dy, x, y if (ctx.act == 1 and ctx.has_res) else None, gamma, beta, save_mean, save_invstd, ctx.act,
                                            ctx.gamma_param, ctx.beta_param, ctx.has_res)
        return dx, None, dg, db, dres, None, None, None, None, None


def _bn_act_backward(dy, x, y, gamma, beta, save_mean, save_invstd, act, gamma_param, beta_param, has_res):
    lib = get_lib()
    C = x.shape[1]
    dy = dy.contiguous(memory_format=_CL)
    dx = torch.empty_like(x, memory_format=_CL)
    dres = torch.empty_like(x, memory_format=_CL) if has_res else None
    red = _ZERO_POOL.acquire(lib.bn_stats_floats(C), x.device)
    dg_t, dg_ret = _grad_target(gamma_param, gamma)
    db_t, db_ret = _grad_target(beta_param, beta)
    PROFILE.bracket("bn_bwd", lambda: lib.bn_act_bwd(dy, y, x, save_mean, save_invstd, gamma, beta, act, x.numel() // C, C, red,
                                                     dx, dres, dg_t, db_t))
    _ZERO_POOL.release(red)
    if dg_ret is None:
        _grad_ready(gamma_param)
    if db_ret is None:
        _grad_ready(beta_param)
    return dx, dg_ret, db_ret, dres


class _BNActEval(torch.autograd.Function):

    @staticmethod
    def forward(ctx, x, gamma, beta, residual, rmean, rvar, act, eps):
        require_cuda(x, gamma, beta)
        N, C, H, W = x.shape
        y = torch.empty_like(x, memory_format=_CL)
        get_lib().bn_act_eval(x, rmean, rvar, gamma, beta, residual, act, N * H * W, C, eps, y)
        ctx.save_for_backward(x, y, gamma, beta, rmean, rvar)
        ctx.act, ctx.eps, ctx.has_res = act, eps, residual is not None
        return y

    @staticmethod
    def backward(ctx, dy):
        x, y, gamma, beta, rmean, rvar = ctx.saved_tensors
        invstd = torch.rsqrt(rvar + ctx.eps).view(1, -1, 1, 1)
        sc = gamma.view(1, -1, 1, 1) * invstd
        if ctx.act == 1:
            g = dy * (y > 0)
        elif ctx.act == 2:
            z = (x - rmean.view(1, -1, 1, 1)) * sc + beta.view(1, -1, 1, 1)
            sg = torch.sigmoid(z)
            g = dy * (sg * (1 + z * (1 - sg)))
        else:
            g = dy
        xhat = (x - rmean.view(1, -1, 1, 1)) * invstd
        return g * sc, (g * xhat).sum((0, 2, 3)), g.sum((0, 2, 3)), (g if ctx.has_res else None), None, None, None, None


def bn_wino_fusable(x, w, bn, stride, pad):
    if os.environ.get("HIFIHR_BN_WINO_FUSE", "1") == "0" or not bn.training or not x.is_cuda:
        return False
    N, C, H, W = x.shape
    K, Cw, R, S = w.shape
    if Cw != C or not _wino_ok(C, K, R, S, stride, pad):
        return False
    lib = get_lib()
    return (_wino_tile(lib, N, H, W, C, K)[0] == 4 and lib.wino_bn_input_supported(C, 4) and lib.wino_bn_input_supported(K, 4)
            and lib.wino_wgrad_parts(N, H, W, C, K, 4) > 0)


class _WinoLink:
    __slots__ = ("lazy", "red", "save_mean", "save_invstd", "gamma", "gamma_param", "beta_param", "g")

    def __init__(self):
        self.lazy, self.red, self.g = False, None, None


class _BNActWinoConv(torch.autograd.Function):

    @staticmethod
    def forward(ctx, x, stats, gamma, beta, residual, w, eps, momentum, running_mean, running_var, want_stats, in_link, link):
        require_cuda(x, stats, gamma, beta, w)
        lib = get_lib()
        x = x.contiguous(memory_format=_CL)
        wk = w.contiguous(memory_format=_CL)
        N, C, H, W = x.shape
        K = wk.shape[0]
        dev = x.device
        tile = _wino_tile(lib, N, H, W, C, K)
        m, P, T = tile
        assert m == 4
        res = residual.contiguous(memory_format=_CL) if residual is not None else None
        out = torch.empty_like(x, memory_format=_CL) if res is not None else None
        save_mean, save_invstd = torch.empty(C, device=dev), torch.empty(C, device=dev)
        U = _WEIGHT_PREP.get(w, wk, 3)
        V = torch.empty(P * T * C, device=dev, dtype=torch.float32)
        y = torch.empty((N, K, H, W), device=dev, dtype=torch.float32, memory_format=_CL)
        stats_next = _ZERO_POOL.acquire(lib.bn_stats_floats(K), dev) if want_stats else None

        def run():
            Uu = U
            if Uu is None:
                Uu = _wino_scratch(dev, "U", P * K * C)
                lib.wino_weight_transform(wk, Uu, K, C, 0, m)
            lib.wino_bn_input_transform(x, stats, gamma, beta, res, out, V, N, H, W, C, m, eps, momentum, save_mean, save_invstd,
                                        running_mean, running_var)
            M = _wino_scratch(dev, "M", P * T * K)
            lib.wino_gemm(V, Uu, M, N, H, W, C, K, ws=_conv_ws(lib, dev, ("wino", N, H, W, C, K, m), False), m=m)
            lib.wino_output_transform(M, y, stats_next, N, H, W, K, m=m)
        if PROFILE.on:
            PROFILE.conv_log.append((("wino", N, H, W, C, K, m), "gemm"))
        PROFILE.bracket("bn_conv_fwd_wino", run)
        _ZERO_POOL.release(stats)
        ctx.save_for_backward(x, out if out is not None else x.new_empty(0), gamma, beta, save_mean, save_invstd, wk, V, y)
        ctx.geom = (N, H, W, C, K, 3, 3, 1, 1)
        ctx.tile = tile
        ctx.has_res = res is not None
        ctx.w_param, ctx.gamma_param, ctx.beta_param = w, gamma, beta
        ctx.in_link, ctx.link = in_link, link
        if in_link is not None:
            in_link.lazy = True
        ctx.set_materialize_grads(False)
        if stats_next is not None:
            ctx.mark_non_differentiable(stats_next)
        return y, stats_next, out

    @staticmethod
    def backward(ctx, gy, _gstats, g_out):
        x, out, gamma, beta, save_mean, save_invstd, wk, V, y = ctx.saved_tensors
        N, H, W, C, K = ctx.geom[:5]
        if gy is None:
            raise NotImplementedError("fused batch-norm + Winograd convolution whose convolution output is unused")
        lib = get_lib()
        dev = x.device
        m, P, T = ctx.tile
        w = ctx.w_param
        need = ctx.needs_input_grad
        gy = gy.contiguous(memory_format=_CL)
        link, in_link = ctx.link, ctx.in_link
        if os.environ.get("HIFIHR_BN_WINO_BWD", "1") == "0":
            d_a, dw, _ = _conv_backward(gy, None, wk, None, V, ctx.geom, w, need_x=True, need_w=need[5])
            if g_out is not None:
                d_a = d_a + g_out
            dx, dg, db, dres = _bn_act_backward(d_a, x, out if ctx.has_res else None, gamma, beta, save_mean, save_invstd, 1,
                                                ctx.gamma_param, ctx.beta_param, ctx.has_res)
            return dx, None, dg, db, dres, dw, None, None, None, None, None, None, None

        res_out = out if ctx.has_res else None
        gadd = g_out.contiguous(memory_format=_CL) if g_out is not None else None
        g_in = torch.empty_like(x, memory_format=_CL)
        red = _ZERO_POOL.acquire(lib.bn_stats_floats(C), dev)
        lazy_in = link.lazy and link.red is not None
        dw_box = [None]
        direct_w = _direct_grad(w, _CL)
        pair = need[5] and m == 4 and _GEMM_PAIR and lib.wino4_bwd_gemm_pair_supported(N, H, W, C, K)

        def run():
            V2 = _wino_scratch(dev, "V", P * T * K)
            Yt = _wino_scratch(dev, "Yt", P * T * K)
            if lazy_in:
                lib.wino_bn_bwd_dual_transform(gy, y, link.save_mean, link.save_invstd, link.gamma, link.red, V2, Yt, N, H, W, K, m,
                                               link.gamma_param.grad, link.beta_param.grad)
            else:
                lib.wino_input_dy_transform(gy, V2, Yt, N, H, W, K, m)
            U2 = _wino_u_bwd(lib, wk, _WEIGHT_PREP.get(w, wk, 4), dev, C, K, m)
            M2 = _wino_scratch(dev, "M", P * T * C)
            slabs = _wino_wgrad_slabs(lib, w, direct_w, False, dev, N, H, W, C, K, m) if need[5] else None
            if pair:
                lib.wino4_bwd_gemm_pair(V2, U2, M2, V, Yt, slabs[0], N, H, W, C, K, slabs[1])
            else:
                lib.wino_gemm(V2, U2, M2, N, H, W, K, C, ws=_conv_ws(lib, dev, ("wino", N, H, W, K, C, m), False), m=m)
            lib.wino_output_transform_bnred(M2, x, res_out, gadd, save_mean, save_invstd, gamma, beta, red, g_in, N, H, W, C, m)
            if need[5]:
                tgt, dw_box[0] = _grad_target(w, wk, _CL)
                _wino_wgrad_tail(lib, V, Yt, slabs, tgt, N, H, W, C, K, m, pair)
        if PROFILE.on:
            if pair:
                PROFILE.conv_log.append((("wino", N, H, W, C, K, m), "gemm-pair"))
            else:
                PROFILE.conv_log.append((("wino", N, H, W, K, C, m), "gemm"))
                PROFILE.conv_log.append((("wino", N, H, W, C, K, m), "gemm-tn"))
        PROFILE.bracket("bn_conv_bwd_wino", run)
        if lazy_in:
            _ZERO_POOL.release(link.red)
            link.red = link.g = None
            link.gamma_param._hifihr_grad_deferred = link.beta_param._hifihr_grad_deferred = False
            _grad_ready(link.gamma_param)
            _grad_ready(link.beta_param)
        if need[5] and direct_w:
            _grad_ready(w)
        dg_ret = db_ret = None
        if in_link is not None and _direct_grad(ctx.gamma_param) and _direct_grad(ctx.beta_param):
            in_link.red, in_link.save_mean, in_link.save_invstd, in_link.gamma = red, save_mean, save_invstd, gamma
            in_link.gamma_param, in_link.beta_param, in_link.g = ctx.gamma_param, ctx.beta_param, g_in
            ctx.gamma_param._hifihr_grad_deferred = ctx.beta_param._hifihr_grad_deferred = True
            dx = g_in
        else:
            dx = torch.empty_like(x, memory_format=_CL)
            dg_t, dg_ret = _grad_target(ctx.gamma_param, gamma)
            db_t, db_ret = _grad_target(ctx.beta_param, beta)
            PROFILE.bracket("bn_bwd", lambda: lib.bn_bwd_apply(g_in, x, save_mean, save_invstd, gamma, N * H * W, C, red, dx, dg_t, db_t))
            _ZERO_POOL.release(red)
            if dg_ret is None:
                _grad_ready(ctx.gamma_param)
            if db_ret is None:
                _grad_ready(ctx.beta_param)
        return dx, None, dg_ret, db_ret, (g_in if ctx.has_res else None), dw_box[0], None, None, None, None, None, None, None


def bn_act_wino_conv(x, stats, bn: torch.nn.BatchNorm2d, residual, w, want_stats):
    link = _WinoLink()
    y, st, out = _BNActWinoConv.apply(x, stats, bn.weight, bn.bias, residual, w, float(bn.eps), float(bn.momentum), bn.running_mean,
                                      bn.running_var, want_stats, getattr(x, "_hifihr_link", None), link)
    y._hifihr_link = link
    return y, st, out


_ACT = {None: 0, False: 0, True: 1, "relu": 1, "swish": 2}


def bn_act(x, stats, bn: torch.nn.BatchNorm2d, residual=None, relu=True):
    act = _ACT[relu]
    if not bn.training:
        assert stats is None, "bn_act in eval mode: the producer was asked for batch statistics (pass want_stats=bn.training)"
        require_cuda(x)
        lib = get_lib()
        xc = x.contiguous(memory_format=_CL)
        N, C, H, W = xc.shape
        res = residual.contiguous(memory_format=_CL) if residual is not None else None
        return _BNActEval.apply(xc, bn.weight, bn.bias, res, bn.running_mean, bn.running_var, act, float(bn.eps))
    if stats is None:
        require_cuda(x)
        lib = get_lib()
        xc = x.contiguous(memory_format=_CL)
        N, C, H, W = xc.shape
        stats = _ZERO_POOL.acquire(lib.bn_stats_floats(C), x.device)
        PROFILE.bracket("bn_stats", lambda: lib.bn_stats(xc, N * H * W, C, stats))
        x = xc
    return _BNAct.apply(x, stats, bn.weight, bn.bias, residual, act, float(bn.eps), float(bn.momentum),
                        bn.running_mean, bn.running_var)


class _BNReluMaxPool(torch.autograd.Function):

    @staticmethod
    def forward(ctx, x, stats, gamma, beta, eps, momentum, running_mean, running_var):
        require_cuda(x, stats, gamma, beta)
        lib = get_lib()
        x = x.contiguous(memory_format=_CL)
        N, C, H, W = x.shape
        OH, OW = (H - 1) // 2 + 1, (W - 1) // 2 + 1
        y = torch.empty((N, C, OH, OW), device=x.device, memory_format=_CL)
        tap = torch.empty(N * OH * OW * C, dtype=torch.uint8, device=x.device)
        save_mean = torch.empty(C, device=x.device)
        save_invstd = torch.empty(C, device=x.device)
        PROFILE.bracket("bn_pool_fwd", lambda: lib.bn_relu_maxpool_fwd(x, stats, gamma, beta, N, H, W, C, eps, momentum, y, tap, save_mean,
                                                                      save_invstd, running_mean, running_var))
        _ZERO_POOL.release(stats)
        ctx.save_for_backward(x, tap, gamma, beta, save_mean, save_invstd, y if _STEM_REDUCE_Y else None)
        ctx.gamma_param, ctx.beta_param = gamma, beta
        return y

    @staticmethod
    def backward(ctx, gy):
        x, tap, gamma, beta, save_mean, save_invstd, y = ctx.saved_tensors
        lib = get_lib()
        N, C, H, W = x.shape
        gy = gy.contiguous(memory_format=_CL)
        _DEFER_DW.flush_early(x.device)
        dx = torch.empty_like(x, memory_format=_CL)
        red = _ZERO_POOL.acquire(lib.bn_stats_floats(C), x.device)
        dg_t, dg_ret = _grad_target(ctx.gamma_param, gamma)
        db_t, db_ret = _grad_target(ctx.beta_param, beta)
        if y is not None:
            PROFILE.bracket("bn_pool_bwd", lambda: lib.bn_relu_maxpool_bwd_y(gy, y, tap, x, save_mean, save_invstd, gamma, beta, N, H, W, C, red, dx,
                                                                            dg_t, db_t))
        else:
            PROFILE.bracket("bn_pool_bwd", lambda: lib.bn_relu_maxpool_bwd(gy, tap, x, save_mean, save_invstd, gamma, beta, N, H, W, C, red, dx,
                                                                          dg_t, db_t))
        _ZERO_POOL.release(red)
        if dg_ret is None:
            _grad_ready(ctx.gamma_param)
        if db_ret is None:
            _grad_ready(ctx.beta_param)
        return dx, None, dg_ret, db_ret, None, None, None, None


def bn_relu_maxpool(x, stats, bn: torch.nn.BatchNorm2d):
    if bn.training and stats is not None and x.is_cuda and os.environ.get("HIFIHR_BN_POOL", "1") != "0":
        N, C, H, W = x.shape
        if get_lib().bn_relu_maxpool_supported(N, H, W, C):
            return _BNReluMaxPool.apply(x, stats, bn.weight, bn.bias, float(bn.eps), float(bn.momentum), bn.running_mean, bn.running_var)
    return maxpool3x3s2(bn_act(x, stats, bn, None, True))


GEOM_TERMS = ("joint_3d", "vert_3d", "edge_length", "mshape", "mpose")
_VF_CACHE = {}


def _vertex_face_csr(faces, V):
    key = (faces.data_ptr(), int(faces.shape[0]), V, str(faces.device))
    hit = _VF_CACHE.get(key)
    if hit is None:
        import numpy as np
        f = faces.detach().cpu().numpy().astype(np.int64)
        flat = f.reshape(-1)
        order = np.argsort(flat, kind="stable")
        off = np.zeros(V + 1, dtype=np.int32)
        np.add.at(off, flat + 1, 1)
        off = np.cumsum(off).astype(np.int32)
        idx = ((order // 3) * 4 + (order % 3)).astype(np.int32)
        hit = (torch.from_numpy(off).to(faces.device), torch.from_numpy(idx).to(faces.device))
        _VF_CACHE[key] = hit
    return hit


class _GeomLoss(torch.autograd.Function):
    @staticmethod
    def forward(ctx, joints, joints_gt, verts, verts_gt, shape, pose, faces, mse, lam):
        require_cuda(joints, verts)
        lib = get_lib()
# ... 743 lines not shown
```

include/hifihr.h:

```cpp
#ifndef HIFIHR_H
#define HIFIHR_H

#include <stddef.h>
#include <stdint.h>

#ifdef __cplusplus
extern "C" {
#endif

#define HIFIHR_OK 0
#define HIFIHR_EINVAL (-1)
#define HIFIHR_EHIP (-2)
#define HIFIHR_ENOMEM (-3)

#define HIFIHR_MANO_NV 778
#define HIFIHR_MANO_NF 1538
#define HIFIHR_MANO_NJ 16

int hifihr_version(void);
const char* hifihr_last_error(void);
int hifihr_device_count(void);

typedef struct hifihr_mano hifihr_mano_t;

// ... 103 lines not shown

int hifihr_adam_step(float* params_d, const float* grads_d, float* exp_avg_d, float* exp_avg_sq_d, size_t n,
                     float grad_scale, float lr, float beta1, float beta2, float eps, float weight_decay, int step,
                     void* stream);
size_t hifihr_adam_state_bytes(void);
int hifihr_adam_step_counted(float* params_d, const float* grads_d, float* exp_avg_d, float* exp_avg_sq_d, size_t n, float grad_scale,
                             float eps, float weight_decay, void* state_d, void* stream);
int hifihr_adam_step_dyn(float* params_d, const float* grads_d, float* exp_avg_d, float* exp_avg_sq_d, size_t n,
                         float grad_scale, float beta1, float beta2, float eps, float weight_decay, const float* dyn_d,
                         void* stream);

size_t hifihr_grad_guard_bytes(void);
size_t hifihr_grad_norm_workspace_bytes(size_t n);
int hifihr_grad_norm(const float* grads_d, size_t n, float grad_scale, float max_norm, void* guard_d, void* ws_d, void* stream);
int hifihr_adam_step_guarded(float* params_d, const float* grads_d, float* exp_avg_d, float* exp_avg_sq_d, size_t n, float grad_scale,
                             float lr, float beta1, float beta2, float eps, float weight_decay, int step, void* state_d,
                             const void* guard_d, void* stream);

size_t hifihr_conv2d_workspace_bytes(int N, int H, int W, int C, int K, int R, int S, int stride, int pad, int bwd_data);
int hifihr_conv2d_fwd(const float* x_d, const float* w_d, const float* bias_d , int act, float* y_d, int N,
                      int H, int W, int C, int K, int R, int S, int stride, int pad, void* ws_d, size_t ws_bytes, void* stream);
int hifihr_bias_relu_bwd(const float* dy_d, const float* y_d, long M, int C, float* g_d, float* db_acc_d ,
                         void* stream);
int hifihr_light_split_fwd(const float* lights_d, int B, float* colors_d, float* directions_d, void* stream);
int hifihr_light_split_bwd(const float* lights_d, const float* gcolors_d, const float* gdirections_d, int B, float* glights_d,
                           void* stream);
int hifihr_conv2d_bwd_data(const float* dy_d, const float* w_d, float* dx_d, float* wt_scratch_d, int N, int H, int W, int C,
                           int K, int R, int S, int stride, int pad, void* ws_d, size_t ws_bytes, void* stream);
int hifihr_conv2d_bwd_weight(const float* x_d, const float* dy_d, float* dw_d, int N, int H, int W, int C, int K, int R, int S,
                             int stride, int pad, void* stream);
size_t hifihr_conv2d_wgrad_workspace_bytes(int N, int H, int W, int C, int K, int R, int S, int stride, int pad);
int hifihr_conv2d_bwd_weight_ws(const float* x_d, const float* dy_d, float* dw_accumulate_d, int N, int H, int W, int C, int K, int R, int S,
                                int stride, int pad, void* ws_d, size_t ws_bytes, void* stream);
int hifihr_conv2d_bwd_weight_c3_supported(int N, int H, int W, int K, int R, int S, int stride, int pad);
int hifihr_conv2d_bwd_weight_c3(const float* x4_d, const float* dy_d, float* dw3_d, int N, int H, int W, int K, int R, int S, int stride,
                                int pad, void* ws_d, size_t ws_bytes, void* stream);
int hifihr_wino_tile(int N, int H, int W, int C, int K);
long hifihr_wino_tiles(int N, int H, int W, int m);
long hifihr_wino_tiles_computed(int N, int H, int W, int m);
size_t hifihr_wino_gemm_workspace_bytes(int N, int H, int W, int C, int K, int m);
int hifihr_wino_wgrad_parts(int N, int H, int W, int C, int K, int m);
int hifihr_wino_weight_transform(const float* w_d, float* u_d, int K, int C, int flip, int m, void* stream);
int hifihr_wino_input_transform(const float* x_d, float* v_d, int N, int H, int W, int C, int m, void* stream);
int hifihr_wino_dy_transform(const float* dy_d, float* yt_d, int N, int H, int W, int K, int m, void* stream);
int hifihr_wino_input_dy_transform(const float* dy_d, float* v_d, float* yt_d, int N, int H, int W, int K, int m, void* stream);
int hifihr_wino_gemm(const float* v_d, const float* u_d, float* m_d, int N, int H, int W, int C, int K, int m, void* ws_d, size_t ws_bytes,
                     void* stream);
int hifihr_wino_output_transform(const float* m_d, float* y_d, float* stats_d , int N, int H, int W, int K, int m, void* stream);
int hifihr_wino_output_transform_act(const float* m_d, float* y_d, const float* bias_d , int act, int N, int H, int W, int K,
                                     int m, void* stream);
int hifihr_wino_output_transform_mask(const float* m_d, float* y_d, const float* mask_d, int N, int H, int W, int K, int m, void* stream);
int hifihr_wino_wgrad_gemm_parts(const float* v_d, const float* yt_d, float* du_parts_d, int N, int H, int W, int C, int K, int parts, int m,
                                 void* stream);
int hifihr_wino_dw_transform_parts(const float* du_parts_d, int parts, float* dw_acc_d, int K, int C, int m, void* stream);
int hifihr_wino_wgrad_gemm(const float* v_d, const float* yt_d, float* du_zeroed_d, int N, int H, int W, int C, int K, void* stream);
int hifihr_wino_dw_transform(float* du_d, float* dw_acc_d, int K, int C, int clear_du ,
                             void* stream);
int hifihr_conv3x3_c64_wino_supported(int N, int H, int W, int C, int K);
int hifihr_zero_page_ready(void* stream);
int hifihr_conv3x3_c64_wino(const float* x_d, const float* u_d, const float* bias_d , int relu, float* y_d,
                            float* stats_d , int N, int H, int W, void* stream);
int hifihr_conv3x3_c64_wino_res(const float* x_d, const float* u_d, const float* res_d, float* y_d, int N, int H, int W, void* stream);
int hifihr_conv3x3_c64_bwd_pair_supported(int N, int H, int W);
int hifihr_conv3x3_c64_bwd_pair(const float* dy_d, const float* u_bwd_d, const float* res_d , float* dx_d, const float* x_d,
                                float* dw_d, void* ws_d, size_t ws_bytes, int N, int H, int W, void* stream);
int hifihr_conv3x3_c64_bwd_pair_slabs(const float* dy_d, const float* u_bwd_d, const float* res_d , float* dx_d, const float* x_d,
                                      void* slabs_d, size_t slab_bytes, int N, int H, int W, int* nslab , void* stream);
typedef struct hifihr_halo_reduce_job {
  const float* slabs_d;
  float* dw_acc_d;
  int nslab;
} hifihr_halo_reduce_job;
int hifihr_conv_halo_wgrad_reduce_multi(const hifihr_halo_reduce_job* jobs , int njobs, void* stream);
int hifihr_wino_bn_input_supported(int C, int m);
int hifihr_wino_bn_input_transform(const float* x_d, float* stats_d, const float* gamma_d, const float* beta_d, const float* residual_d,
                                   float* out_d, float* v_d, int N, int H, int W, int C, int m, float eps, float momentum,
                                   float* save_mean_d, float* save_invstd_d, float* running_mean_d, float* running_var_d, void* stream);
int hifihr_wino_output_transform_bnred(const float* m_d, const float* x_d, const float* out_d , const float* gadd_d ,
                                       const float* save_mean_d, const float* save_invstd_d, const float* gamma_d, const float* beta_d,
                                       float* red_d, float* g_d, int N, int H, int W, int C, int m, void* stream);
int hifihr_wino_bn_bwd_dual_transform(const float* g_d, const float* y_d, const float* save_mean_d, const float* save_invstd_d,
                                      const float* gamma_d, float* red_d, float* v_d, float* yt_d, int N, int H, int W, int K, int m,
                                      float* dgamma_acc_d, float* dbeta_acc_d, void* stream);
int hifihr_bn_bwd_apply(const float* g_d, const float* x_d, const float* save_mean_d, const float* save_invstd_d, const float* gamma_d, long M,
                        int C, float* red_d, float* dx_d, float* dgamma_acc_d, float* dbeta_acc_d, void* stream);
int hifihr_wino4_bwd_gemm_pair_supported(int N, int H, int W, int C, int K);
int hifihr_wino4_bwd_gemm_pair(const float* V2_d, const float* U2_d, float* M2_d, const float* Vx_d, const float* Yt_d, float* dU_parts_d,
                               int N, int H, int W, int C, int K, int parts, void* stream);
typedef struct hifihr_wino_dw_job {
  const float* du_parts_d;
  float* dw_acc_d;
  int parts, K, C;
} hifihr_wino_dw_job;
int hifihr_wino4_dw_transform_multi(const hifihr_wino_dw_job* jobs, int njobs, void* stream);
size_t hifihr_bgemm_nt_workspace_bytes(int M, int N, int K, int batch);
int hifihr_bgemm_nt(const float* a_d, const float* b_d, float* c_d, int M, int N, int K, int batch,
                    void* ws_d , size_t ws_bytes, void* stream);
int hifihr_bgemm_tn_parts(int M, int N, int T, int batch);
int hifihr_bgemm_describe(int tn, int M, int N, int K_or_T, int batch, char* out, int cap);
int hifihr_bgemm_tn(const float* a_d, const float* b_d, float* c_parts_d, int M, int N, int T, int batch, int parts, void* stream);
int hifihr_weight_transpose(const float* w_d, float* wt_d, int K, int RS, int C, void* stream);
int hifihr_conv2d_bwd_data_pre(const float* dy_d, const float* wt_d, float* dx_d, int N, int H, int W, int C, int K, int R, int S,
                               int stride, int pad, void* ws_d, size_t ws_bytes, void* stream);
int hifihr_conv2d_bwd_data_pre_res(const float* dy_d, const float* wt_d, const float* res_d, float* dx_d, int N, int H, int W, int C, int K,
                                   int R, int S, int stride, int pad, void* ws_d, size_t ws_bytes, void* stream);
int hifihr_conv2d_bwd_data_pre_plus1x1_supported(int N, int H, int W, int C, int K, int R, int S, int stride, int pad);
int hifihr_conv2d_bwd_data_pre_plus1x1(const float* dy_d, const float* wt_d, const float* dy2_d, const float* wt2_d, float* dx_d, int N, int H,
                                       int W, int C, int K, int R, int S, int stride, int pad, void* stream);
int hifihr_conv2d_bwd_weight_plus1x1_supported(int N, int H, int W, int C, int K, int R, int S, int stride, int pad);
int hifihr_conv2d_bwd_weight_plus1x1(const float* x_d, const float* dy_d, float* dw_d, const float* dy2_d, float* dw2_d, int N, int H, int W,
                                     int C, int K, int R, int S, int stride, int pad, void* stream);
typedef struct hifihr_prep_job {
  const float* src;
  float* dst;
  int K, C, RS, kind;
} hifihr_prep_job;
int hifihr_weight_prep(const hifihr_prep_job* jobs_d, int njobs, int blocks_per_job, void* stream);

int hifihr_conv2d_describe(int N, int H, int W, int C, int K, int R, int S, int stride, int pad, int direction, char* out, int cap);

int hifihr_conv2d_fwd_bnstats(const float* x_d, const float* w_d, float* y_d, float* stats_d, int N, int H, int W, int C, int K,
                              int R, int S, int stride, int pad, void* ws_d, size_t ws_bytes, void* stream);
int hifihr_conv2d_fwd_bnstats_pair_supported(int N, int H, int W, int C, int stride, int K1, int R1, int pad1, int K2, int R2, int pad2);
int hifihr_conv2d_fwd_bnstats_pair(const float* x_d, const float* w1_d, float* y1_d, float* stats1_d, int K1, int R1, int pad1, const float* w2_d,
                                   float* y2_d, float* stats2_d, int K2, int R2, int pad2, int N, int H, int W, int C, int stride, void* stream);

int hifihr_bn_stats_floats(int C);
int hifihr_bn_stats(const float* x_d, long M, int C, float* stats_d, void* stream);
int hifihr_bn_act_fwd(const float* x_d, float* stats_d , const float* gamma_d, const float* beta_d,
                      const float* residual_d , int act, long M, int C, float eps, float momentum, float* y_d,
                      float* save_mean_d, float* save_invstd_d, float* running_mean_d, float* running_var_d, void* stream);
int hifihr_bn_act_eval(const float* x_d, const float* running_mean_d, const float* running_var_d, const float* gamma_d, const float* beta_d,
                       const float* residual_d , int act, long M, int C, float eps, float* y_d, void* stream);
int hifihr_bn_act_bwd(const float* dy_d, const float* y_d , const float* x_d, const float* save_mean_d,
                      const float* save_invstd_d, const float* gamma_d, const float* beta_d , int act, long M, int C,
                      float* red_scratch_d, float* dx_d, float* dres_d, float* dgamma_acc_d, float* dbeta_acc_d, void* stream);

int hifihr_bn_relu_maxpool_supported(int N, int H, int W, int C);
int hifihr_bn_relu_maxpool_fwd(const float* x_d, float* stats_d, const float* gamma_d, const float* beta_d, int N, int H, int W, int C,
                               float eps, float momentum, float* pooled_d, unsigned char* tap_d, float* save_mean_d, float* save_invstd_d,
                               float* running_mean_d, float* running_var_d, void* stream);
int hifihr_bn_relu_maxpool_bwd(const float* pooled_grad_d, const unsigned char* tap_d, const float* x_d, const float* save_mean_d,
                               const float* save_invstd_d, const float* gamma_d, const float* beta_d, int N, int H, int W, int C,
                               float* red_scratch_d, float* dx_d, float* dgamma_acc_d, float* dbeta_acc_d, void* stream);
int hifihr_bn_relu_maxpool_bwd_y(const float* pooled_grad_d, const float* pooled_d, const unsigned char* tap_d, const float* x_d,
                                 const float* save_mean_d, const float* save_invstd_d, const float* gamma_d, const float* beta_d, int N, int H, int W,
                                 int C, float* red_scratch_d, float* dx_d, float* dgamma_acc_d, float* dbeta_acc_d, void* stream);

int hifihr_dwconv2d_fwd(const float* x_d, const float* w_d, float* y_d, float* stats_d , int N, int H, int W, int C,
                        int OH, int OW, int K, int stride, int pad_top, int pad_left, void* stream);
int hifihr_dwconv2d_bwd_data(const float* dy_d, const float* w_d, float* dx_d, int N, int H, int W, int C, int OH, int OW, int K,
                             int stride, int pad_top, int pad_left, void* stream);
int hifihr_dwconv2d_bwd_weight(const float* x_d, const float* dy_d, float* dw_d, int N, int H, int W, int C, int OH, int OW,
                               int K, int stride, int pad_top, int pad_left, void* stream);
int hifihr_dwconv2d_fwd_bnswish(const float* x_d, const float* mean_d, const float* invstd_d, const float* gamma_d, const float* beta_d,
                                const float* w_d, float* y_d, float* stats_d , int N, int H, int W, int C, int OH, int OW,
                                int K, int stride, int pad_top, int pad_left, void* stream);
int hifihr_dwconv2d_bwd_weight_bnswish(const float* x_d, const float* mean_d, const float* invstd_d, const float* gamma_d,
                                       const float* beta_d, const float* dy_d, float* dw_d, int N, int H, int W, int C, int OH, int OW,
                                       int K, int stride, int pad_top, int pad_left, void* stream);
int hifihr_bn_finalize_fwd(float* stats_d, long M, int C, float eps, float momentum, float* save_mean_d, float* save_invstd_d,
                           float* running_mean_d , float* running_var_d , void* stream);

int hifihr_mmpool_fwd(const float* x_d, const float* p_d, int B, int HW, int C, float* y_d, int* argmax_d, float* xmax_d,
                      float* xavg_d, void* stream);
int hifihr_mmpool_bwd(const float* gy_d, const float* p_d, const int* argmax_d, const float* xmax_d, const float* xavg_d, int B,
// ... 130 lines not shown
```

Measured before the change: 6731 images/sec.

## Fuse downsample-branch batch-norm into Winograd BN input and output transforms

Adds fused kernels that apply the downsample shortcut's batch-norm (scale/shift from its stats) inside the residual BN+ReLU Winograd input transform, and computes the downsample BN's backward reduction in the same output-transform pass. The standalone downsample BN forward pass and part of its backward are removed, cutting full-tensor reads and writes and kernel launches in ResNet-18's downsample blocks. It also links BN outputs to their sole consumer so the residual BN reduction can be fused in backward. Default mode is 'bwd', which adds complexity and more autograd plumbing.

```diff
diff --git a/hifihr_amd/_lib.py b/hifihr_amd/_lib.py
--- a/hifihr_amd/_lib.py
+++ b/hifihr_amd/_lib.py
@@ -210,6 +210,9 @@
         c.hifihr_wino_bn_input_supported.argtypes = [c_int, c_int]
         c.hifihr_wino_bn_input_transform.argtypes = [_c_float_p] * 7 + [c_int] * 5 + [c_float, c_float] + [_c_float_p] * 4 + [c_void_p]
         c.hifihr_wino_output_transform_bnred.argtypes = [_c_float_p] * 10 + [c_int] * 5 + [c_void_p]
+        c.hifihr_wino_bn_input_transform_ds.argtypes = ([_c_float_p] * 10 + [c_int] * 5 + [c_float, c_float] + [_c_float_p] * 4 + [c_float, c_float]
+                                                        + [_c_float_p] * 4 + [c_void_p])
+        c.hifihr_wino_output_transform_bnred_ds.argtypes = [_c_float_p] * 14 + [c_int] * 5 + [c_void_p]
         c.hifihr_wino_bn_bwd_dual_transform.argtypes = [_c_float_p] * 8 + [c_int] * 5 + [_c_float_p] * 2 + [c_void_p]
         c.hifihr_bn_bwd_apply.argtypes = [_c_float_p] * 5 + [c_long, c_int] + [_c_float_p] * 4 + [c_void_p]
         c.hifihr_joint_terms_fwd.argtypes = [_c_float_p] * 4 + [c_int] * 3 + [POINTER(c_float), _c_float_p, c_void_p]
@@ -620,6 +623,22 @@
                                                              _fp(beta), _fp(red), _fp(g), N, H, W, C, m, _stream_of(Mm)),
                    "hifihr_wino_output_transform_bnred")
 
+    def wino_bn_input_transform_ds(self, x, stats, gamma, beta, yds, ds_stats, ds_gamma, ds_beta, out, V, N, H, W, C, m, eps, momentum, save_mean,
+                                   save_invstd, running_mean, running_var, ds_eps, ds_momentum, ds_save_mean, ds_save_invstd, ds_running_mean,
+                                   ds_running_var):
+        self.check(self.c.hifihr_wino_bn_input_transform_ds(_fp(x), _fp(stats), _fp(gamma), _fp(beta), _fp(yds), _fp(ds_stats), _fp(ds_gamma),
+                                                            _fp(ds_beta), _fp(out), _fp(V), N, H, W, C, m, eps, momentum, _fp(save_mean),
+                                                            _fp(save_invstd), _fp(running_mean), _fp(running_var), ds_eps, ds_momentum,
+                                                            _fp(ds_save_mean), _fp(ds_save_invstd), _fp(ds_running_mean), _fp(ds_running_var),
+                                                            _stream_of(x)), "hifihr_wino_bn_input_transform_ds")
+
+    def wino_output_transform_bnred_ds(self, Mm, x, out, gadd, save_mean, save_invstd, gamma, beta, red, g, yds, ds_save_mean, ds_save_invstd,
+                                       red_ds, N, H, W, C, m):
+        self.check(self.c.hifihr_wino_output_transform_bnred_ds(_fp(Mm), _fp(x), _fp(out), _fp(gadd), _fp(save_mean), _fp(save_invstd),
+                                                                _fp(gamma), _fp(beta), _fp(red), _fp(g), _fp(yds), _fp(ds_save_mean),
+                                                                _fp(ds_save_invstd), _fp(red_ds), N, H, W, C, m, _stream_of(Mm)),
+                   "hifihr_wino_output_transform_bnred_ds")
+
     def wino_bn_bwd_dual_transform(self, g, y, save_mean, save_invstd, gamma, red, V, Yt, N, H, W, K, m, dgamma_acc, dbeta_acc):
         self.check(self.c.hifihr_wino_bn_bwd_dual_transform(_fp(g), _fp(y), _fp(save_mean), _fp(save_invstd), _fp(gamma), _fp(red), _fp(V), _fp(Yt),
                                                             N, H, W, K, m, _fp(dgamma_acc), _fp(dbeta_acc), _stream_of(g)),
diff --git a/hifihr_amd/csrc/bn_fold.h b/hifihr_amd/csrc/bn_fold.h
--- a/hifihr_amd/csrc/bn_fold.h
+++ b/hifihr_amd/csrc/bn_fold.h
@@ -68,6 +68,36 @@
   mu = (float)m;
   var = v > 0.0 ? (float)v : 0.f;
 }
+template <int NS>
+__device__ __forceinline__ void slot_sums_fwd2_n(const double* __restrict__ bufA, const double* __restrict__ bufB, int C, int c, double (&s)[4]) {
+  double a[NS], b[NS], e[NS], f[NS];
+#pragma unroll
+  for (int sl = 0; sl < NS; ++sl) {
+    a[sl] = bufA[(size_t)sl * 2 * C + c]; b[sl] = bufA[(size_t)sl * 2 * C + C + c];
+    e[sl] = bufB[(size_t)sl * 2 * C + c]; f[sl] = bufB[(size_t)sl * 2 * C + C + c];
+  }
+  s[0] = s[1] = s[2] = s[3] = 0.0;
+#pragma unroll
+  for (int sl = 0; sl < NS; ++sl) { s[0] += a[sl]; s[1] += b[sl]; s[2] += e[sl]; s[3] += f[sl]; }
+}
+__device__ __forceinline__ void slot_mean_var2(const float* __restrict__ statsA, const float* __restrict__ statsB, int C, int c, long M, float& muA,
+                                               float& varA, float& muB, float& varB) {
+  const int ns = stat_slots_used(C);
+  if (ns == kStatSlots) {
+    slot_mean_var(statsA, C, c, M, muA, varA);
+    slot_mean_var(statsB, C, c, M, muB, varB);
+    return;
+  }
+  const double* bufA = reinterpret_cast<const double*>(statsA);
+  const double* bufB = reinterpret_cast<const double*>(statsB);
+  double s[4];
+  if (ns == 16) { HIFIHR_NO_HOIST(); slot_sums_fwd2_n<16>(bufA, bufB, C, c, s); }
+  else { HIFIHR_NO_HOIST(); slot_sums_fwd2_n<8>(bufA, bufB, C, c, s); }
+  const double mA = s[0] / (double)M, mB = s[2] / (double)M;
+  const double vA = s[1] / (double)M - mA * mA, vB = s[3] / (double)M - mB * mB;
+  muA = (float)mA; varA = vA > 0.0 ? (float)vA : 0.f;
+  muB = (float)mB; varB = vB > 0.0 ? (float)vB : 0.f;
+}
 __device__ __forceinline__ void clear_slots_fwd(float* __restrict__ stats, int C, unsigned* __restrict__ cnt) {
   float4* p = reinterpret_cast<float4*>(stats);
   const int n4 = stat_slots_used(C) * 2 * C / 2;
diff --git a/hifihr_amd/csrc/hifihr_api.hip b/hifihr_amd/csrc/hifihr_api.hip
--- a/hifihr_amd/csrc/hifihr_api.hip
+++ b/hifihr_amd/csrc/hifihr_api.hip
@@ -1628,6 +1628,36 @@
   return HIFIHR_OK;
 }
 
+int hifihr_wino_bn_input_transform_ds(const float* x, float* stats, const float* gamma, const float* beta, const float* yds, float* ds_stats,
+                                      const float* ds_gamma, const float* ds_beta, float* out, float* V, int N, int H, int W, int C, int m,
+                                      float eps, float momentum, float* save_mean, float* save_invstd, float* running_mean, float* running_var,
+                                      float ds_eps, float ds_momentum, float* ds_save_mean, float* ds_save_invstd, float* ds_running_mean,
+                                      float* ds_running_var, void* stream) {
+  if (!x || !stats || !gamma || !beta || !yds || !ds_stats || !ds_gamma || !ds_beta || !out || !V || !save_mean || !save_invstd ||
+      !ds_save_mean || !ds_save_invstd || ds_stats == stats || N <= 0 || H <= 0 || W <= 0 ||
+      ((running_mean == nullptr) != (running_var == nullptr)) || ((ds_running_mean == nullptr) != (ds_running_var == nullptr)))
+    return fail(HIFIHR_EINVAL, "hifihr_wino_bn_input_transform_ds: bad argument");
+  if (!hifihr_wino_bn_input_supported(C, m)) return fail(HIFIHR_EINVAL, "hifihr_wino_bn_input_transform_ds: needs m = 4 and C % 4 == 0, C <= 512");
+  HIP_TRY(hifihr::launch_wino4_bn_input_transform_ds(x, stats, gamma, beta, yds, ds_stats, ds_gamma, ds_beta, out, V, N, H, W, C, eps, momentum,
+                                                     save_mean, save_invstd, running_mean, running_var, ds_eps, ds_momentum, ds_save_mean,
+                                                     ds_save_invstd, ds_running_mean, ds_running_var, (hipStream_t)stream));
+  return HIFIHR_OK;
+}
+
+int hifihr_wino_output_transform_bnred_ds(const float* Mm, const float* x, const float* out, const float* gadd, const float* save_mean,
+                                          const float* save_invstd, const float* gamma, const float* beta, float* red, float* g, const float* yds,
+                                          const float* ds_save_mean, const float* ds_save_invstd, float* red_ds, int N, int H, int W, int C, int m,
+                                          void* stream) {
+  if (!Mm || !x || !out || !save_mean || !save_invstd || !gamma || !beta || !red || !g || !yds || !ds_save_mean || !ds_save_invstd || !red_ds ||
+      red_ds == red || N <= 0 || H <= 0 || W <= 0)
+    return fail(HIFIHR_EINVAL, "hifihr_wino_output_transform_bnred_ds: bad argument");
+  if (!hifihr_wino_bn_input_supported(C, m))
+    return fail(HIFIHR_EINVAL, "hifihr_wino_output_transform_bnred_ds: needs m = 4 and C % 4 == 0, C <= 512");
+  HIP_TRY(hifihr::launch_wino4_output_transform_bnred_ds(Mm, x, out, gadd, save_mean, save_invstd, gamma, beta, red, g, yds, ds_save_mean,
+                                                         ds_save_invstd, red_ds, N, H, W, C, (hipStream_t)stream));
+  return HIFIHR_OK;
+}
+
 int hifihr_wino_bn_bwd_dual_transform(const float* g, const float* y, const float* save_mean, const float* save_invstd, const float* gamma,
                                       float* red, float* V, float* Yt, int N, int H, int W, int K, int m, float* dgamma_acc, float* dbeta_acc,
                                       void* stream) {
diff --git a/hifihr_amd/csrc/hifihr_internal.h b/hifihr_amd/csrc/hifihr_internal.h
--- a/hifihr_amd/csrc/hifihr_internal.h
+++ b/hifihr_amd/csrc/hifihr_internal.h
@@ -445,6 +445,15 @@
 hipError_t launch_wino4_output_transform_bnred(const float* Mm, const float* x, const float* outp, const float* gadd, const float* save_mean,
                                                const float* save_invstd, const float* gamma, const float* beta, float* red, float* g, int N,
                                                int H, int W, int C, hipStream_t st);
+hipError_t launch_wino4_bn_input_transform_ds(const float* x, float* stats, const float* gamma, const float* beta, const float* y_ds,
+                                              float* stats_ds, const float* gamma_ds, const float* beta_ds, float* out, float* V, int N, int H,
+                                              int W, int C, float eps, float momentum, float* save_mean, float* save_invstd,
+                                              float* running_mean, float* running_var, float eps_ds, float momentum_ds, float* save_mean_ds,
+                                              float* save_invstd_ds, float* running_mean_ds, float* running_var_ds, hipStream_t st);
+hipError_t launch_wino4_output_transform_bnred_ds(const float* Mm, const float* x, const float* outp, const float* gadd, const float* save_mean,
+                                                  const float* save_invstd, const float* gamma, const float* beta, float* red, float* g,
+                                                  const float* y_ds, const float* ds_mean, const float* ds_invstd, float* red_ds, int N, int H,
+                                                  int W, int C, hipStream_t st);
 hipError_t launch_wino4_bn_bwd_dual_transform(const float* g, const float* y, const float* save_mean, const float* save_invstd, const float* gamma,
                                               float* red, float* V, float* Y, int N, int H, int W, int K, float* dgamma_acc, float* dbeta_acc,
                                               hipStream_t st);
diff --git a/hifihr_amd/csrc/wino4_bn.hip b/hifihr_amd/csrc/wino4_bn.hip
--- a/hifihr_amd/csrc/wino4_bn.hip
+++ b/hifihr_amd/csrc/wino4_bn.hip
@@ -65,11 +65,12 @@
   }
 }
 
-template <bool RES, typename T>
-__device__ __forceinline__ void wbn_emit(const WbnPatch<RES, T>& p, const float* s_sc, const float* s_sh, float* __restrict__ out,
-                                         float* __restrict__ V, int C, size_t Tn) {
+template <bool RES, bool DS, typename T>
+__device__ __forceinline__ void wbn_emit(const WbnPatch<RES, T>& p, const float* s_sc, const float* s_sh, const float* s_sc2,
+                                         const float* s_sh2, float* __restrict__ out, float* __restrict__ V, int C, size_t Tn) {
   constexpr int VW = VecWidth<T>::n;
   const T sc = ldT<T>(&s_sc[p.cg * VW]), sh = ldT<T>(&s_sh[p.cg * VW]);
+  const T sc2 = DS ? ldT<T>(&s_sc2[p.cg * VW]) : zeroT<T>(), sh2 = DS ? ldT<T>(&s_sh2[p.cg * VW]) : zeroT<T>();
   T tt[6][6];
 #pragma unroll
   for (int c = 0; c < 6; ++c) {
@@ -77,7 +78,9 @@
 #pragma unroll
     for (int r = 0; r < 6; ++r) {
       const bool ok = (p.ok >> (6 * r + c)) & 1ull;
-      const T a = bn_res_relu<T>(p.v[r][c], sc, sh, RES ? p.r[RES ? r : 0][RES ? c : 0] : zeroT<T>(), RES);
+      T idt = RES ? p.r[RES ? r : 0][RES ? c : 0] : zeroT<T>();
+      if (DS) idt = idt * sc2 + sh2;
+      const T a = bn_res_relu<T>(p.v[r][c], sc, sh, idt, RES);
       col[r] = ok ? a : zeroT<T>();
       if (RES && r >= 1 && r <= 4 && c >= 1 && c <= 4 && ok)
         stT(out + p.own[RES ? r - 1 : 0][RES ? c - 1 : 0] * C + p.cg * VW, a);
@@ -96,60 +99,101 @@
   }
 }
 
-template <bool RES, typename T, bool MOS>
+constexpr int kWbnNoRes = 0, kWbnRes = 1, kWbnResDs = 2;
+
+struct WbnDsBn {
+  float* stats;
+  const float* gamma;
+  const float* beta;
+  float eps, momentum;
+  float* save_mean;
+  float* save_invstd;
+  float* running_mean;
+  float* running_var;
+};
+
+__device__ __forceinline__ void wbn_table(float mu, float var, const float* __restrict__ gamma, const float* __restrict__ beta, int c, long M,
+                                          float eps, float momentum, float* s_sc, float* s_sh, float* __restrict__ save_mean,
+                                          float* __restrict__ save_invstd, float* __restrict__ running_mean, float* __restrict__ running_var) {
+  const float is = 1.0f / sqrtf(var + eps);
+  const float sc = is * gamma[c];
+  s_sc[c] = sc;
+  s_sh[c] = beta[c] - mu * sc;
+  if (blockIdx.x == 0) {
+    save_mean[c] = mu;
+    save_invstd[c] = is;
+    if (running_mean) {
+      running_mean[c] = (1.f - momentum) * running_mean[c] + momentum * mu;
+      const float unbiased = (M > 1) ? var * ((float)M / (float)(M - 1)) : var;
+      running_var[c] = (1.f - momentum) * running_var[c] + momentum * unbiased;
+    }
+  }
+}
+
+template <int RES, typename T, bool MOS>
 __global__ __launch_bounds__(256) void wino4_bn_input_transform_kernel(const float* __restrict__ x, float* __restrict__ stats,
                                                                          const float* __restrict__ gamma, const float* __restrict__ beta,
                                                                          const float* __restrict__ res, float* __restrict__ out,
                                                                          float* __restrict__ V, TileGeo geo, int C,
                                                                          float eps, float momentum, float* __restrict__ save_mean,
                                                                          float* __restrict__ save_invstd, float* __restrict__ running_mean,
-                                                                         float* __restrict__ running_var) {
+                                                                         float* __restrict__ running_var, WbnDsBn ds) {
+  constexpr bool HAS_RES = RES != kWbnNoRes, DS = RES == kWbnResDs;
   if (!MOS) geo.G = 0;
   __shared__ float s_sc[kWbnMaxC], s_sh[kWbnMaxC];
+  __shared__ float s_sc2[DS ? kWbnMaxC : 1], s_sh2[DS ? kWbnMaxC : 1];
   const long M = (long)geo.N * geo.H * geo.W;
   const size_t Tn = tile_count(geo), total = Tn * (C / VecWidth<T>::n);
-  for (int c = threadIdx.x; c < C; c += 256) {
-    float mu, var;
-    slot_mean_var(stats, C, c, M, mu, var);
-    const float is = 1.0f / sqrtf(var + eps);
-    const float sc = is * gamma[c];
-    s_sc[c] = sc;
-    s_sh[c] = beta[c] - mu * sc;
-    if (blockIdx.x == 0) {
-      save_mean[c] = mu;
-      save_invstd[c] = is;
-      if (running_mean) {
-        running_mean[c] = (1.f - momentum) * running_mean[c] + momentum * mu;
-        const float unbiased = (M > 1) ? var * ((float)M / (float)(M - 1)) : var;
-        running_var[c] = (1.f - momentum) * running_var[c] + momentum * unbiased;
-      }
+  if (DS && 2 * C > 256) {
+    for (int c = threadIdx.x; c < C; c += 256) {
+      float mu, var, mu2, var2;
+      slot_mean_var2(stats, ds.stats, C, c, M, mu, var, mu2, var2);
+      wbn_table(mu, var, gamma, beta, c, M, eps, momentum, s_sc, s_sh, save_mean, save_invstd, running_mean, running_var);
+      wbn_table(mu2, var2, ds.gamma, ds.beta, c, M, ds.eps, ds.momentum, s_sc2, s_sh2, ds.save_mean, ds.save_invstd, ds.running_mean,
+                ds.running_var);
+    }
+  } else {
+    for (int j = threadIdx.x; j < (DS ? 2 * C : C); j += 256) {
+      const bool second = DS && j >= C;
+      const int c = second ? j - C : j;
+      float mu, var;
+      slot_mean_var(second ? ds.stats : stats, C, c, M, mu, var);
+      if (!second) wbn_table(mu, var, gamma, beta, c, M, eps, momentum, s_sc, s_sh, save_mean, save_invstd, running_mean, running_var);
+      else wbn_table(mu, var, ds.gamma, ds.beta, c, M, ds.eps, ds.momentum, s_sc2, s_sh2, ds.save_mean, ds.save_invstd, ds.running_mean,
+                     ds.running_var);
     }
   }
   __syncthreads();
   for (size_t i = (size_t)blockIdx.x * 256 + threadIdx.x; i < total; i += (size_t)gridDim.x * 256) {
-    WbnPatch<RES, T> p;
-    wbn_load<RES, T>(p, i, x, res, geo, C);
-    wbn_emit<RES, T>(p, s_sc, s_sh, out, V, C, Tn);
+    WbnPatch<HAS_RES, T> p;
+    wbn_load<HAS_RES, T>(p, i, x, res, geo, C);
+    wbn_emit<HAS_RES, DS, T>(p, s_sc, s_sh, s_sc2, s_sh2, out, V, C, Tn);
   }
   unsigned* cnt = stat_fwd_counters(stats, C);
-  if (last_workgroup(cnt)) clear_slots_fwd(stats, C, cnt);
-}
-
-template <bool RES, bool ADD, bool MOS>
+  if (last_workgroup(cnt)) {
+    clear_slots_fwd(stats, C, cnt);
+    if (DS) clear_slots_fwd(ds.stats, C, stat_fwd_counters(ds.stats, C));
+  }
+}
+
+template <bool RES, bool ADD, bool MOS, bool DS>
 __global__ __launch_bounds__(256) void wino4_output_transform_bnred_kernel(const float* __restrict__ Mm, const float* __restrict__ x,
                                                                           const float* __restrict__ outp, const float* __restrict__ gadd,
                                                                           const float* __restrict__ save_mean, const float* __restrict__ save_invstd,
                                                                           const float* __restrict__ gamma, const float* __restrict__ beta,
-                                                                          float* __restrict__ red, float* __restrict__ g, TileGeo geo, int C) {
+                                                                          float* __restrict__ red, float* __restrict__ g, TileGeo geo, int C,
+                                                                          const float* __restrict__ y_ds, const float* __restrict__ ds_mean,
+                                                                          const float* __restrict__ ds_invstd, float* __restrict__ red_ds) {
   if (!MOS) geo.G = 0;
-  __shared__ float4 redl[2][16][16];
+  __shared__ float4 redl[DS ? 3 : 2][16][16];
   const int cl = threadIdx.x & 15, tl = threadIdx.x >> 4;
   const int k = blockIdx.y * 64 + cl * 4;
   const bool kok = k < C;
   const size_t T = tile_count(geo);
-  V4 sg = zero4(), sq = zero4();
+  V4 sg = zero4(), sq = zero4(), sq2 = zero4();
   if (kok) {
     const V4 mu = ld4(save_mean + k), is = ld4(save_invstd + k), ga = ld4(gamma + k), be = ld4(beta + k);
+    const V4 mu2 = DS ? ld4(ds_mean + k) : zero4(), is2 = DS ? ld4(ds_invstd + k) : zero4();
     const V4 sc = V4{is.x * ga.x, is.y * ga.y, is.z * ga.z, is.w * ga.w};
     const V4 sh = V4{be.x - mu.x * sc.x, be.y - mu.y * sc.y, be.z - mu.z * sc.z, be.w - mu.w * sc.w};
     for (size_t t = (size_t)blockIdx.x * 16 + tl; t < T; t += (size_t)gridDim.x * 16) {
@@ -173,7 +217,7 @@
       for (int a = 0; a < 4; ++a) {
         const AxisPx ry = row_px(geo, at, by_, a);
         if (ry.ok) {
-          V4 xv[4], ov[4], av[4];
+          V4 xv[4], ov[4], av[4], yv[4];
           bool ok[4];
           size_t ob[4];
 #pragma unroll
@@ -183,6 +227,7 @@
             xv[b] = ld4(x + o);
             ov[b] = RES ? ld4(outp + o) : zero4();
             av[b] = ADD ? ld4(gadd + o) : zero4();
+            yv[b] = DS ? ld4(y_ds + o) : zero4();
           }
           V4 o[4];
           at6(s[a], o);
@@ -199,6 +244,10 @@
               sg = sg + gm;
               sq.x += gm.x * ((xv[b].x - mu.x) * is.x); sq.y += gm.y * ((xv[b].y - mu.y) * is.y);
               sq.z += gm.z * ((xv[b].z - mu.z) * is.z); sq.w += gm.w * ((xv[b].w - mu.w) * is.w);
+              if (DS) {
+                sq2.x += gm.x * ((yv[b].x - mu2.x) * is2.x); sq2.y += gm.y * ((yv[b].y - mu2.y) * is2.y);
+                sq2.z += gm.z * ((yv[b].z - mu2.z) * is2.z); sq2.w += gm.w * ((yv[b].w - mu2.w) * is2.w);
+              }
             }
           }
         }
@@ -206,17 +255,27 @@
     }
   }
   redl[0][tl][cl] = make_float4(sg.x, sg.y, sg.z, sg.w); redl[1][tl][cl] = make_float4(sq.x, sq.y, sq.z, sq.w);
+  if (DS) redl[DS ? 2 : 0][tl][cl] = make_float4(sq2.x, sq2.y, sq2.z, sq2.w);
   __syncthreads();
   if (tl == 0 && kok) {
-    float4 a1 = redl[0][0][cl], a2 = redl[1][0][cl];
+    float4 a1 = redl[0][0][cl], a2 = redl[1][0][cl], a3 = DS ? redl[DS ? 2 : 0][0][cl] : make_float4(0.f, 0.f, 0.f, 0.f);
     for (int r = 1; r < 16; ++r) {
       const float4 b1 = redl[0][r][cl], b2 = redl[1][r][cl];
       a1 = make_float4(a1.x + b1.x, a1.y + b1.y, a1.z + b1.z, a1.w + b1.w);
       a2 = make_float4(a2.x + b2.x, a2.y + b2.y, a2.z + b2.z, a2.w + b2.w);
+      if (DS) {
+        const float4 b3 = redl[DS ? 2 : 0][r][cl];
+        a3 = make_float4(a3.x + b3.x, a3.y + b3.y, a3.z + b3.z, a3.w + b3.w);
+      }
     }
     float* sp = red + (size_t)(blockIdx.x & (stat_slots_used(C) - 1)) * 2 * C;
     atomicAdd(sp + k, a1.x); atomicAdd(sp + k + 1, a1.y); atomicAdd(sp + k + 2, a1.z); atomicAdd(sp + k + 3, a1.w);
     atomicAdd(sp + C + k, a2.x); atomicAdd(sp + C + k + 1, a2.y); atomicAdd(sp + C + k + 2, a2.z); atomicAdd(sp + C + k + 3, a2.w);
+    if (DS) {
+      float* sp2 = red_ds + (size_t)(blockIdx.x & (stat_slots_used(C) - 1)) * 2 * C;
+      atomicAdd(sp2 + k, a1.x); atomicAdd(sp2 + k + 1, a1.y); atomicAdd(sp2 + k + 2, a1.z); atomicAdd(sp2 + k + 3, a1.w);
+      atomicAdd(sp2 + C + k, a3.x); atomicAdd(sp2 + C + k + 1, a3.y); atomicAdd(sp2 + C + k + 2, a3.z); atomicAdd(sp2 + C + k + 3, a3.w);
+    }
   }
 }
 
@@ -313,43 +372,78 @@
 
 bool wino4_bn_supported(int C) { return C >= 4 && C % 4 == 0 && C <= kWbnMaxC; }
 
+static hipError_t wbn_input_launch(const float* x, float* stats, const float* gamma, const float* beta, const float* res, float* out,
+                                   float* V, int N, int H, int W, int C, float eps, float momentum, float* save_mean, float* save_invstd,
+                                   float* running_mean, float* running_var, const WbnDsBn* ds, hipStream_t st) {
+  if (!wino4_bn_supported(C) || ((res == nullptr) != (out == nullptr)) || (ds != nullptr && res == nullptr)) return hipErrorInvalidValue;
+  const TileGeo geo = wino4_geo(N, H, W);
+  const size_t total = tile_count(geo) * (C / 4);
+  const WbnDsBn dsv = ds ? *ds : WbnDsBn{};
+#define HIFIHR_WBN_IN2(R_, M_)                                                                                                                 \
+  hipLaunchKernelGGL((wino4_bn_input_transform_kernel<R_, V4, M_>), dim3(wbn_grid(total)), dim3(256), 0, st, x, stats, gamma, beta, res, out, V, \
+                     geo, C, eps, momentum, save_mean, save_invstd, running_mean, running_var, dsv)
+#define HIFIHR_WBN_IN(R_) { if (geo.G) HIFIHR_WBN_IN2(R_, true); else HIFIHR_WBN_IN2(R_, false); }
+  if (ds != nullptr) HIFIHR_WBN_IN(kWbnResDs) else if (res != nullptr) HIFIHR_WBN_IN(kWbnRes) else HIFIHR_WBN_IN(kWbnNoRes)
+#undef HIFIHR_WBN_IN
+#undef HIFIHR_WBN_IN2
+  return hipGetLastError();
+}
+
 hipError_t launch_wino4_bn_input_transform(const float* x, float* stats, const float* gamma, const float* beta, const float* res, float* out,
                                            float* V, int N, int H, int W, int C, float eps, float momentum, float* save_mean,
                                            float* save_invstd, float* running_mean, float* running_var, hipStream_t st) {
-  if (!wino4_bn_supported(C) || ((res == nullptr) != (out == nullptr))) return hipErrorInvalidValue;
-  const TileGeo geo = wino4_geo(N, H, W);
-  const size_t total = tile_count(geo) * (C / 4);
-#define HIFIHR_WBN_IN2(R_, M_)                                                                                                                 \
-  hipLaunchKernelGGL((wino4_bn_input_transform_kernel<R_, V4, M_>), dim3(wbn_grid(total)), dim3(256), 0, st, x, stats, gamma, beta, res, out, V, \
-                     geo, C, eps, momentum, save_mean, save_invstd, running_mean, running_var)
-#define HIFIHR_WBN_IN(R_) { if (geo.G) HIFIHR_WBN_IN2(R_, true); else HIFIHR_WBN_IN2(R_, false); }
-  if (res != nullptr) HIFIHR_WBN_IN(true) else HIFIHR_WBN_IN(false)
-#undef HIFIHR_WBN_IN
-#undef HIFIHR_WBN_IN2
-  return hipGetLastError();
-}
-
-hipError_t launch_wino4_output_transform_bnred(const float* Mm, const float* x, const float* outp, const float* gadd, const float* save_mean,
-                                               const float* save_invstd, const float* gamma, const float* beta, float* red, float* g, int N,
-                                               int H, int W, int C, hipStream_t st) {
-  if (!wino4_bn_supported(C)) return hipErrorInvalidValue;
+  return wbn_input_launch(x, stats, gamma, beta, res, out, V, N, H, W, C, eps, momentum, save_mean, save_invstd, running_mean, running_var,
+                          nullptr, st);
+}
+
+hipError_t launch_wino4_bn_input_transform_ds(const float* x, float* stats, const float* gamma, const float* beta, const float* y_ds,
+                                              float* stats_ds, const float* gamma_ds, const float* beta_ds, float* out, float* V, int N, int H,
+                                              int W, int C, float eps, float momentum, float* save_mean, float* save_invstd,
+                                              float* running_mean, float* running_var, float eps_ds, float momentum_ds, float* save_mean_ds,
+                                              float* save_invstd_ds, float* running_mean_ds, float* running_var_ds, hipStream_t st) {
+  if (y_ds == nullptr || stats_ds == nullptr || stats_ds == stats) return hipErrorInvalidValue;
+  const WbnDsBn ds{stats_ds, gamma_ds, beta_ds, eps_ds, momentum_ds, save_mean_ds, save_invstd_ds, running_mean_ds, running_var_ds};
+  return wbn_input_launch(x, stats, gamma, beta, y_ds, out, V, N, H, W, C, eps, momentum, save_mean, save_invstd, running_mean, running_var,
+                          &ds, st);
+}
+
+static hipError_t wbn_bnred_launch(const float* Mm, const float* x, const float* outp, const float* gadd, const float* save_mean,
+                                   const float* save_invstd, const float* gamma, const float* beta, float* red, float* g, int N, int H, int W,
+                                   int C, const float* y_ds, const float* ds_mean, const float* ds_invstd, float* red_ds, hipStream_t st) {
+  if (!wino4_bn_supported(C) || (y_ds != nullptr && outp == nullptr)) return hipErrorInvalidValue;
   const TileGeo geo = wino4_geo(N, H, W);
   const size_t T = tile_count(geo);
   size_t bx = (T + 15) / 16;
   if (bx > 1024) bx = 1024;
   const dim3 grid((unsigned)bx, (C + 63) / 64);
-#define HIFIHR_BNRED2(R_, A_, M_)                                                                                                          \
-  hipLaunchKernelGGL((wino4_output_transform_bnred_kernel<R_, A_, M_>), grid, dim3(256), 0, st, Mm, x, outp, gadd, save_mean, save_invstd, gamma, \
-                     beta, red, g, geo, C)
-#define HIFIHR_BNRED(R_, A_) { if (geo.G) HIFIHR_BNRED2(R_, A_, true); else HIFIHR_BNRED2(R_, A_, false); }
-  if (outp != nullptr) {
-    if (gadd != nullptr) HIFIHR_BNRED(true, true) else HIFIHR_BNRED(true, false)
+#define HIFIHR_BNRED2(R_, A_, M_, D_)                                                                                                      \
+  hipLaunchKernelGGL((wino4_output_transform_bnred_kernel<R_, A_, M_, D_>), grid, dim3(256), 0, st, Mm, x, outp, gadd, save_mean, save_invstd, \
+                     gamma, beta, red, g, geo, C, y_ds, ds_mean, ds_invstd, red_ds)
+#define HIFIHR_BNRED(R_, A_, D_) { if (geo.G) HIFIHR_BNRED2(R_, A_, true, D_); else HIFIHR_BNRED2(R_, A_, false, D_); }
+  if (y_ds != nullptr) {
+    if (gadd != nullptr) HIFIHR_BNRED(true, true, true) else HIFIHR_BNRED(true, false, true)
+  } else if (outp != nullptr) {
+    if (gadd != nullptr) HIFIHR_BNRED(true, true, false) else HIFIHR_BNRED(true, false, false)
   } else {
-    if (gadd != nullptr) HIFIHR_BNRED(false, true) else HIFIHR_BNRED(false, false)
+    if (gadd != nullptr) HIFIHR_BNRED(false, true, false) else HIFIHR_BNRED(false, false, false)
   }
 #undef HIFIHR_BNRED
 #undef HIFIHR_BNRED2
   return hipGetLastError();
+}
+
+hipError_t launch_wino4_output_transform_bnred(const float* Mm, const float* x, const float* outp, const float* gadd, const float* save_mean,
+                                               const float* save_invstd, const float* gamma, const float* beta, float* red, float* g, int N,
+                                               int H, int W, int C, hipStream_t st) {
+  return wbn_bnred_launch(Mm, x, outp, gadd, save_mean, save_invstd, gamma, beta, red, g, N, H, W, C, nullptr, nullptr, nullptr, nullptr, st);
+}
+
+hipError_t launch_wino4_output_transform_bnred_ds(const float* Mm, const float* x, const float* outp, const float* gadd, const float* save_mean,
+                                                  const float* save_invstd, const float* gamma, const float* beta, float* red, float* g,
+                                                  const float* y_ds, const float* ds_mean, const float* ds_invstd, float* red_ds, int N, int H,
+                                                  int W, int C, hipStream_t st) {
+  if (y_ds == nullptr || ds_mean == nullptr || ds_invstd == nullptr || red_ds == nullptr || red_ds == red) return hipErrorInvalidValue;
+  return wbn_bnred_launch(Mm, x, outp, gadd, save_mean, save_invstd, gamma, beta, red, g, N, H, W, C, y_ds, ds_mean, ds_invstd, red_ds, st);
 }
 
 hipError_t launch_wino4_bn_bwd_dual_transform(const float* g, const float* y, const float* save_mean, const float* save_invstd, const float* gamma,
diff --git a/hifihr_amd/network.py b/hifihr_amd/network.py
--- a/hifihr_amd/network.py
+++ b/hifihr_amd/network.py
@@ -62,12 +62,15 @@
 
 class _PendingBN:
 
-    def __init__(self, y, stats, bn, identity):
-        self.y, self.stats, self.bn, self.identity = y, stats, bn, identity
+    def __init__(self, y, stats, bn, identity, ds=None):
+        self.y, self.stats, self.bn, self.identity, self.ds = y, stats, bn, identity, ds
 
     def materialize(self):
         from . import ops
-        return ops.bn_act(self.y, self.stats, self.bn, self.identity, True)
+        idt = self.identity
+        if self.ds is not None:
+            idt = ops.bn_act(self.ds[0], self.ds[1], self.ds[2], None, False)
+        return ops.bn_act(self.y, self.stats, self.bn, idt, True)
 
 
 def _resolve(x):
@@ -93,7 +96,10 @@
         if isinstance(x, _PendingBN):
             p = x
             if p.bn.training and ops.bn_wino_fusable(p.y, self.conv1.weight, p.bn, self.conv1.stride, self.conv1.pad):
-                out, st, x = ops.bn_act_wino_conv(p.y, p.stats, p.bn, p.identity, self.conv1.weight, self.bn1.training)
+                if p.ds is not None:
+                    out, st, x = ops.bn_act_wino_conv(p.y, p.stats, p.bn, None, self.conv1.weight, self.bn1.training, p.ds)
+                else:
+                    out, st, x = ops.bn_act_wino_conv(p.y, p.stats, p.bn, p.identity, self.conv1.weight, self.bn1.training)
                 fused = True
             else:
                 x = p.materialize()
@@ -110,11 +116,16 @@
             out = ops.bn_act(out, st, self.bn1, None, True)
             out, st = _conv_bn(self.conv2, out, self.bn2)
         idt = x
+        if idt_raw is None and self.downsample is not None:
+            idt_raw, st_ds = _conv_bn(self.downsample[0], x, self.downsample[1])
         if idt_raw is not None:
+            if (self.lazy_out and self.bn2.training and st_ds is not None and st is not None and idt_raw.is_cuda
+                    and ops.bn_ds_fuse_mode() in ("1", "fwd")):
+                return _PendingBN(out, st, self.bn2, None, (idt_raw, st_ds, self.downsample[1]))
             idt = ops.bn_act(idt_raw, st_ds, self.downsample[1], None, False)
-        elif self.downsample is not None:
-            idt, st2 = _conv_bn(self.downsample[0], x, self.downsample[1])
-            idt = ops.bn_act(idt, st2, self.downsample[1], None, False)
+            bn_link = getattr(idt, "_hifihr_bn_link", None)
+            if bn_link is not None and self.lazy_out and self.bn2.training:
+                bn_link.sole_consumer = True
         if self.lazy_out and self.bn2.training:
             return _PendingBN(out, st, self.bn2, idt)
         return ops.bn_act(out, st, self.bn2, idt, True)
diff --git a/hifihr_amd/ops.py b/hifihr_amd/ops.py
--- a/hifihr_amd/ops.py
+++ b/hifihr_amd/ops.py
@@ -1258,9 +1258,16 @@
     return os.environ.get("HIFIHR_CONV_FORK", "1") != "0"
 
 
+class _BNLink:
+    __slots__ = ("sole_consumer", "x", "save_mean", "save_invstd", "red")
+
+    def __init__(self):
+        self.sole_consumer, self.x, self.save_mean, self.save_invstd, self.red = False, None, None, None, None
+
+
 class _BNAct(torch.autograd.Function):
     @staticmethod
-    def forward(ctx, x, stats, gamma, beta, residual, act, eps, momentum, running_mean, running_var):
+    def forward(ctx, x, stats, gamma, beta, residual, act, eps, momentum, running_mean, running_var, link=None):
         require_cuda(x, stats, gamma, beta)
         lib = get_lib()
         x = x.contiguous(memory_format=_CL)
@@ -1276,14 +1283,34 @@
         ctx.save_for_backward(x, y if (act == 1 and residual is not None) else x.new_empty(0), gamma, beta, save_mean, save_invstd)
         ctx.act, ctx.has_res, ctx.M, ctx.C = act, residual is not None, M, C
         ctx.gamma_param, ctx.beta_param = gamma, beta
+        ctx.link = link
+        if link is not None:
+            link.x, link.save_mean, link.save_invstd = x, save_mean, save_invstd
         return y
 
     @staticmethod
     def backward(ctx, dy):
         x, y, gamma, beta, save_mean, save_invstd = ctx.saved_tensors
+        link = ctx.link
+        if link is not None and link.red is not None:
+            red, link.red = link.red, None
+            link.x = link.save_mean = link.save_invstd = None
+            dy = dy.contiguous(memory_format=_CL)
+            dx = torch.empty_like(x, memory_format=_CL)
+            dg_t, dg = _grad_target(ctx.gamma_param, gamma)
+            db_t, db = _grad_target(ctx.beta_param, beta)
+            PROFILE.bracket("bn_bwd", lambda: get_lib().bn_bwd_apply(dy, x, save_mean, save_invstd, gamma, ctx.M, ctx.C, red, dx, dg_t, db_t))
+            _ZERO_POOL.release(red)
+            if dg is None:
+                _grad_ready(ctx.gamma_param)
+            if db is None:
+                _grad_ready(ctx.beta_param)
+            return dx, None, dg, db, None, None, None, None, None, None, None
+        if link is not None:
+            link.x = link.save_mean = link.save_invstd = None
         dx, dg, db, dres = _bn_act_backward(dy, x, y if (ctx.act == 1 and ctx.has_res) else None, gamma, beta, save_mean, save_invstd, ctx.act,
                                             ctx.gamma_param, ctx.beta_param, ctx.has_res)
-        return dx, None, dg, db, dres, None, None, None, None, None
+        return dx, None, dg, db, dres, None, None, None, None, None, None
 
 
 def _bn_act_backward(dy, x, y, gamma, beta, save_mean, save_invstd, act, gamma_param, beta_param, has_res):
@@ -1356,7 +1383,8 @@
 class _BNActWinoConv(torch.autograd.Function):
 
     @staticmethod
-    def forward(ctx, x, stats, gamma, beta, residual, w, eps, momentum, running_mean, running_var, want_stats, in_link, link):
+    def forward(ctx, x, stats, gamma, beta, residual, w, eps, momentum, running_mean, running_var, want_stats, in_link, link,
+                ds_raw=None, ds_stats=None, ds_gamma=None, ds_beta=None, ds_bn=None, res_link=None):
         require_cuda(x, stats, gamma, beta, w)
         lib = get_lib()
         x = x.contiguous(memory_format=_CL)
@@ -1368,6 +1396,13 @@
         m, P, T = tile
         assert m == 4
         res = residual.contiguous(memory_format=_CL) if residual is not None else None
+        ds = ds_raw is not None
+        if ds:
+            assert res is None and ds_raw.shape == x.shape
+            res = ds_raw = ds_raw.contiguous(memory_format=_CL)
+            ds_mean, ds_invstd = torch.empty(C, device=dev), torch.empty(C, device=dev)
+            ds_eps, ds_momentum, ds_rmean, ds_rvar = ds_bn
+        ds_in = ds
         out = torch.empty_like(x, memory_format=_CL) if res is not None else None
         save_mean, save_invstd = torch.empty(C, device=dev), torch.empty(C, device=dev)
         U = _WEIGHT_PREP.get(w, wk, 3)
@@ -1380,8 +1415,13 @@
             if Uu is None:
                 Uu = _wino_scratch(dev, "U", P * K * C)
                 lib.wino_weight_transform(wk, Uu, K, C, 0, m)
-            lib.wino_bn_input_transform(x, stats, gamma, beta, res, out, V, N, H, W, C, m, eps, momentum, save_mean, save_invstd,
-                                        running_mean, running_var)
+            if ds_in:
+                lib.wino_bn_input_transform_ds(x, stats, gamma, beta, res, ds_stats, ds_gamma, ds_beta, out, V, N, H, W, C, m, eps, momentum,
+                                               save_mean, save_invstd, running_mean, running_var, ds_eps, ds_momentum, ds_mean, ds_invstd,
+                                               ds_rmean, ds_rvar)
+            else:
+                lib.wino_bn_input_transform(x, stats, gamma, beta, res, out, V, N, H, W, C, m, eps, momentum, save_mean, save_invstd,
+                                            running_mean, running_var)
             M = _wino_scratch(dev, "M", P * T * K)
             lib.wino_gemm(V, Uu, M, N, H, W, C, K, ws=_conv_ws(lib, dev, ("wino", N, H, W, C, K, m), False), m=m)
             lib.wino_output_transform(M, y, stats_next, N, H, W, K, m=m)
@@ -1389,11 +1429,17 @@
             PROFILE.conv_log.append((("wino", N, H, W, C, K, m), "gemm"))
         PROFILE.bracket("bn_conv_fwd_wino", run)
         _ZERO_POOL.release(stats)
-        ctx.save_for_backward(x, out if out is not None else x.new_empty(0), gamma, beta, save_mean, save_invstd, wk, V, y)
+        if ds:
+            _ZERO_POOL.release(ds_stats)
+        ctx.save_for_backward(x, out if out is not None else x.new_empty(0), gamma, beta, save_mean, save_invstd, wk, V, y,
+                              *((ds_raw, ds_gamma, ds_beta, ds_mean, ds_invstd) if ds else ()))
         ctx.geom = (N, H, W, C, K, 3, 3, 1, 1)
         ctx.tile = tile
         ctx.has_res = res is not None
+        ctx.ds, ctx.ds_bwd = ds, ds and bn_ds_fuse_mode() == "1"
+        ctx.res_link = res_link if (res_link is not None and not ds and res is not None) else None
         ctx.w_param, ctx.gamma_param, ctx.beta_param = w, gamma, beta
+        ctx.ds_gamma_param, ctx.ds_beta_param = ds_gamma, ds_beta
         ctx.in_link, ctx.link = in_link, link
         if in_link is not None:
             in_link.lazy = True
@@ -1404,7 +1450,10 @@
 
     @staticmethod
     def backward(ctx, gy, _gstats, g_out):
-        x, out, gamma, beta, save_mean, save_invstd, wk, V, y = ctx.saved_tensors
+        x, out, gamma, beta, save_mean, save_invstd, wk, V, y = ctx.saved_tensors[:9]
+        ds = ctx.ds
+        if ds:
+            ds_raw, ds_gamma, ds_beta, ds_mean, ds_invstd = ctx.saved_tensors[9:]
         N, H, W, C, K = ctx.geom[:5]
         if gy is None:
             raise NotImplementedError("fused batch-norm + Winograd convolution whose convolution output is unused")
@@ -1421,12 +1470,20 @@
                 d_a = d_a + g_out
             dx, dg, db, dres = _bn_act_backward(d_a, x, out if ctx.has_res else None, gamma, beta, save_mean, save_invstd, 1,
                                                 ctx.gamma_param, ctx.beta_param, ctx.has_res)
-            return dx, None, dg, db, dres, dw, None, None, None, None, None, None, None
+            if ds:
+                d_ds, dg_ds, db_ds, _ = _bn_act_backward(dres, ds_raw, None, ds_gamma, ds_beta, ds_mean, ds_invstd, 0, ctx.ds_gamma_param,
+                                                         ctx.ds_beta_param, False)
+                return dx, None, dg, db, None, dw, None, None, None, None, None, None, None, d_ds, None, dg_ds, db_ds, None, None
+            return dx, None, dg, db, dres, dw, None, None, None, None, None, None, None, None, None, None, None, None, None
 
         res_out = out if ctx.has_res else None
         gadd = g_out.contiguous(memory_format=_CL) if g_out is not None else None
         g_in = torch.empty_like(x, memory_format=_CL)
         red = _ZERO_POOL.acquire(lib.bn_stats_floats(C), dev)
+        rl = ctx.res_link
+        if rl is not None and rl.x is None:
+            rl = None
+        red_ds = _ZERO_POOL.acquire(lib.bn_stats_floats(C), dev) if (ctx.ds_bwd or rl is not None) else None
         lazy_in = link.lazy and link.red is not None
         dw_box = [None]
         direct_w = _direct_grad(w, _CL)
@@ -1447,7 +1504,14 @@
                 lib.wino4_bwd_gemm_pair(V2, U2, M2, V, Yt, slabs[0], N, H, W, C, K, slabs[1])
             else:
                 lib.wino_gemm(V2, U2, M2, N, H, W, K, C, ws=_conv_ws(lib, dev, ("wino", N, H, W, K, C, m), False), m=m)
-            lib.wino_output_transform_bnred(M2, x, res_out, gadd, save_mean, save_invstd, gamma, beta, red, g_in, N, H, W, C, m)
+            if ctx.ds_bwd:
+                lib.wino_output_transform_bnred_ds(M2, x, res_out, gadd, save_mean, save_invstd, gamma, beta, red, g_in, ds_raw, ds_mean, ds_invstd,
+                                                   red_ds, N, H, W, C, m)
+            elif rl is not None:
+                lib.wino_output_transform_bnred_ds(M2, x, res_out, gadd, save_mean, save_invstd, gamma, beta, red, g_in, rl.x, rl.save_mean,
+                                                   rl.save_invstd, red_ds, N, H, W, C, m)
+            else:
+                lib.wino_output_transform_bnred(M2, x, res_out, gadd, save_mean, save_invstd, gamma, beta, red, g_in, N, H, W, C, m)
             if need[5]:
                 tgt, dw_box[0] = _grad_target(w, wk, _CL)
                 _wino_wgrad_tail(lib, V, Yt, slabs, tgt, N, H, W, C, K, m, pair)
@@ -1482,13 +1546,45 @@
                 _grad_ready(ctx.gamma_param)
             if db_ret is None:
                 _grad_ready(ctx.beta_param)
-        return dx, None, dg_ret, db_ret, (g_in if ctx.has_res else None), dw_box[0], None, None, None, None, None, None, None
-
-
-def bn_act_wino_conv(x, stats, bn: torch.nn.BatchNorm2d, residual, w, want_stats):
+        if rl is not None:
+            rl.red = red_ds
+        if not ds:
+            return (dx, None, dg_ret, db_ret, (g_in if ctx.has_res else None), dw_box[0], None, None, None, None, None, None, None,
+                    None, None, None, None, None, None)
+        if ctx.ds_bwd:
+            d_ds = torch.empty_like(x, memory_format=_CL)
+            dg_t, dg_ds = _grad_target(ctx.ds_gamma_param, ds_gamma)
+            db_t, db_ds = _grad_target(ctx.ds_beta_param, ds_beta)
+            PROFILE.bracket("bn_bwd", lambda: lib.bn_bwd_apply(g_in, ds_raw, ds_mean, ds_invstd, ds_gamma, N * H * W, C, red_ds, d_ds, dg_t, db_t))
+            _ZERO_POOL.release(red_ds)
+            if dg_ds is None:
+                _grad_ready(ctx.ds_gamma_param)
+            if db_ds is None:
+                _grad_ready(ctx.ds_beta_param)
+        else:
+            d_ds, dg_ds, db_ds, _ = _bn_act_backward(g_in, ds_raw, None, ds_gamma, ds_beta, ds_mean, ds_invstd, 0, ctx.ds_gamma_param,
+                                                     ctx.ds_beta_param, False)
+        return dx, None, dg_ret, db_ret, None, dw_box[0], None, None, None, None, None, None, None, d_ds, None, dg_ds, db_ds, None, None
+
+
+def bn_ds_fuse_mode():
+    v = os.environ.get("HIFIHR_BN_DS_FUSE", "bwd")
+    return v if v in ("0", "fwd", "1") else "bwd"
+
+
+def bn_act_wino_conv(x, stats, bn: torch.nn.BatchNorm2d, residual, w, want_stats, ds=None):
     link = _WinoLink()
+    ds_args = (None, None, None, None, None)
+    res_link = getattr(residual, "_hifihr_bn_link", None) if residual is not None else None
+    if res_link is not None and not (res_link.sole_consumer and bn_ds_fuse_mode() in ("1", "bwd")
+                                     and os.environ.get("HIFIHR_BN_WINO_BWD", "1") != "0"):
+        res_link = None
+    if ds is not None:
+        assert residual is None
+        ds_raw, ds_stats, ds_bn = ds
+        ds_args = (ds_raw, ds_stats, ds_bn.weight, ds_bn.bias, (float(ds_bn.eps), float(ds_bn.momentum), ds_bn.running_mean, ds_bn.running_var))
     y, st, out = _BNActWinoConv.apply(x, stats, bn.weight, bn.bias, residual, w, float(bn.eps), float(bn.momentum), bn.running_mean,
-                                      bn.running_var, want_stats, getattr(x, "_hifihr_link", None), link)
+                                      bn.running_var, want_stats, getattr(x, "_hifihr_link", None), link, *ds_args, res_link)
     y._hifihr_link = link
     return y, st, out
 
@@ -1514,6 +1610,11 @@
         stats = _ZERO_POOL.acquire(lib.bn_stats_floats(C), x.device)
         PROFILE.bracket("bn_stats", lambda: lib.bn_stats(xc, N * H * W, C, stats))
         x = xc
+    if act == 0 and residual is None and x.shape[1] % 4 == 0 and x.shape[1] <= 512:
+        link = _BNLink()
+        y = _BNAct.apply(x, stats, bn.weight, bn.bias, None, act, float(bn.eps), float(bn.momentum), bn.running_mean, bn.running_var, link)
+        y._hifihr_bn_link = link
+        return y
     return _BNAct.apply(x, stats, bn.weight, bn.bias, residual, act, float(bn.eps), float(bn.momentum),
                         bn.running_mean, bn.running_var)
 
diff --git a/include/hifihr.h b/include/hifihr.h
--- a/include/hifihr.h
+++ b/include/hifihr.h
@@ -209,6 +209,15 @@
 int hifihr_wino_bn_bwd_dual_transform(const float* g_d, const float* y_d, const float* save_mean_d, const float* save_invstd_d,
                                       const float* gamma_d, float* red_d, float* v_d, float* yt_d, int N, int H, int W, int K, int m,
                                       float* dgamma_acc_d, float* dbeta_acc_d, void* stream);
+int hifihr_wino_bn_input_transform_ds(const float* x_d, float* stats_d, const float* gamma_d, const float* beta_d, const float* yds_d,
+                                      float* ds_stats_d, const float* ds_gamma_d, const float* ds_beta_d, float* out_d, float* v_d, int N, int H,
+                                      int W, int C, int m, float eps, float momentum, float* save_mean_d, float* save_invstd_d,
+                                      float* running_mean_d, float* running_var_d, float ds_eps, float ds_momentum, float* ds_save_mean_d,
+                                      float* ds_save_invstd_d, float* ds_running_mean_d, float* ds_running_var_d, void* stream);
+int hifihr_wino_output_transform_bnred_ds(const float* m_d, const float* x_d, const float* out_d, const float* gadd_d ,
+                                          const float* save_mean_d, const float* save_invstd_d, const float* gamma_d, const float* beta_d,
+                                          float* red_d, float* g_d, const float* yds_d, const float* ds_save_mean_d,
+                                          const float* ds_save_invstd_d, float* red_ds_d, int N, int H, int W, int C, int m, void* stream);
 int hifihr_bn_bwd_apply(const float* g_d, const float* x_d, const float* save_mean_d, const float* save_invstd_d, const float* gamma_d, long M,
                         int C, float* red_d, float* dx_d, float* dgamma_acc_d, float* dbeta_acc_d, void* stream);
 int hifihr_wino4_bwd_gemm_pair_supported(int N, int H, int W, int C, int K);
```

Result: no change. 6750 images/sec (median of 6 runs) (+0.3%).
